# Academich/translation-transformer

Measured on AMD Instinct MI355X. Metric: reactions/sec (SMILES decoded), greedy speculative, higher is better.
Workload: dtype f32

## Files before the change

### include/ttx.h

```cpp
#ifndef TTX_H
#define TTX_H

#include <stdint.h>

#ifdef __cplusplus
extern "C" {
#endif

#define TTX_ABI_VERSION 4

typedef enum ttx_status {
  TTX_OK = 0,
  TTX_ERR_INVALID = -1,
  TTX_ERR_HIP = -2,
  TTX_ERR_NO_DEVICE = -3,
  TTX_ERR_REFERENCE = -4,
  TTX_ERR_NOMEM = -5,
  TTX_ERR_ROW_REPLAY = -6,
  TTX_ERR_MAX_STEPS = -7
} ttx_status;

typedef struct ttx_config {
  int32_t vocab_size;
  int32_t src_vocab_size;
// ... 244 lines not shown
  int32_t max_len, beam_size;
  float   temperature;
  int32_t pad_token, bos_token, eos_token;
  uint64_t seed;
} ttx_sbs_params;
typedef struct ttx_sbs_trace {
  int32_t* d_parent; int32_t* d_token;
  float* d_phi; float* d_g;
} ttx_sbs_trace;
int ttx_sbs_generate(ttx_session* s, const int64_t* d_src, int B, int Ls, const int64_t* d_row_keys, const ttx_sbs_params* p,
                     int64_t* d_out, float* d_logp, float* d_gumbel, const ttx_sbs_trace* trace_or_null,
                     ttx_beam_search_stats* stats, void* stream);

typedef struct ttx_sbs_filter {
  int32_t top_k;
  float   top_p;
} ttx_sbs_filter;
int ttx_sbs_generate_ex(ttx_session* s, const int64_t* d_src, int B, int Ls, const int64_t* d_row_keys, const ttx_sbs_params* p,
                        const ttx_sbs_filter* f_or_null, const int64_t* d_prefix, int ld_prefix, const int32_t* h_prefix_len,
                        int64_t* d_out, float* d_logp, float* d_gumbel, const ttx_sbs_trace* trace_or_null,
                        ttx_beam_search_stats* stats, void* stream);
int ttx_sbs_generate_bias(ttx_session* s, const int64_t* d_src, int B, int Ls, const int64_t* d_row_keys, const ttx_sbs_params* p,
                          const ttx_sbs_filter* f_or_null, const int64_t* d_prefix, int ld_prefix, const int32_t* h_prefix_len,
                          const float* d_bias, int ld_bias, int64_t* d_out, float* d_logp, float* d_gumbel,
                          const ttx_sbs_trace* trace_or_null, ttx_beam_search_stats* stats, void* stream);

typedef struct ttx_sbs_pool_stats {
  int64_t model_calls;
  int64_t running_rows;
  int64_t src_tokens_padded;
  int64_t live_slots;
  double  decode_ms;
  int32_t status;
  int32_t pad_;
  int32_t* d_src_running_rows;
} ttx_sbs_pool_stats;
int ttx_sbs_generate_pool(ttx_session** sessions, int n_sessions, const int64_t* d_src, int S_total, int Ls_all,
                          const int32_t* h_len, const int64_t* d_row_keys, int capacity ,
                          const ttx_sbs_params* p, const ttx_sbs_filter* f_or_null,
                          const int64_t* d_prefix, int ld_prefix, const int32_t* h_prefix_len,
                          int64_t* d_out , float* d_logp, float* d_gumbel ,
                          ttx_sbs_pool_stats* stats, void* stream);

int ttx_greedy_speculative_generate_many(ttx_session** sessions, int n_sessions, int n_batches,
                                         const int64_t* const* d_src, const int* B, const int* Ls,
                                         const ttx_gen_params* p, int64_t* const* d_out, ttx_gen_stats* stats,
                                         void* stream);

int ttx_greedy_speculative_generate_rows(ttx_session** sessions, int n_sessions, int n_batches,
                                         const int64_t* const* d_src, const int* B, const int* Ls,
                                         const ttx_gen_params* p, int64_t* const* d_out, int16_t* const* d_traj,
                                         int32_t* const* d_fin_step, ttx_gen_stats* stats, void* stream);

int ttx_greedy_speculative_generate_pool(ttx_session** sessions, int n_sessions, const int64_t* d_src, int R_total, int Ls_all,
                                         const int32_t* h_len, int capacity, const ttx_gen_params* p, int64_t* d_out,
                                         int16_t* d_traj, int32_t* d_fin_step, ttx_gen_stats* stats, void* stream);

typedef struct ttx_tokenizer ttx_tokenizer;
int  ttx_tokenizer_create(const char* const* tokens, const int32_t* ids, int n, ttx_tokenizer** out);
void ttx_tokenizer_destroy(ttx_tokenizer* t);
int  ttx_tokenizer_encode(const ttx_tokenizer* t, const char* line, int32_t* out, int cap);
int  ttx_tokenizer_encode_batch(const ttx_tokenizer* t, const char* const* lines, int B, int64_t* out, int cap_cols);
int  ttx_tokenizer_decode(const ttx_tokenizer* t, const int64_t* ids, int n, char* out, int cap);

int ttx_debug_step_snapshot(ttx_session* s, int32_t* info, float* h_logits, int32_t* h_act, int32_t* h_front,
                            int32_t* h_gen);

int ttx_last_kernel_profile(ttx_session* s, double* gemm_ms, int64_t* gemm_launches, double* empty_pair_ms);

int ttx_debug_gemm_bench(ttx_session* s, int M, int N, int K, int splits, int variant, int reps, double* us_per_launch,
                         double* max_abs_diff);

int ttx_debug_gemm(ttx_session* s, const float* d_x, int ldx, const float* d_w, int ldw, const float* d_bias, float* d_y, int ldy,
                   const int32_t* d_m, int m_max, int N, int K, int relu, int splits, int64_t slab_stride, int variant, int tiling,
                   int32_t* kernel_id, void* stream);
int ttx_debug_gemm_act(ttx_session* s, const float* d_x, int ldx, const float* d_w, int ldw, const float* d_bias, float* d_y, int ldy,
                       const int32_t* d_m, int m_max, int N, int K, int activation, int splits, int64_t slab_stride, int variant,
                       int tiling, int32_t* kernel_id, void* stream);

int ttx_debug_finish_ln(ttx_session* s, const float* d_slabs, int n_slabs, int64_t slab_stride, const float* d_bias,
                        const float* d_resid, const float* d_g1, const float* d_b1, const float* d_g2, const float* d_b2,
                        const uint8_t* d_row_valid, float* d_y, const int32_t* d_m, int m_max, int d, float eps, void* stream);

int ttx_debug_attn(ttx_session* s, const float* d_q, int ldq, const float* d_k, const float* d_v, int ldkv, float* d_out, int H,
                   float scale, int L, int Lk, const int32_t* d_tok, int pad, const uint8_t* d_key_pad, const int32_t* d_mem_row,
                   const int32_t* d_act_idx, const int32_t* d_front, const int32_t* d_src_of, const int32_t* d_src_len,
                   const float* d_kcache, const float* d_vcache, int64_t cache_seq_stride, const int32_t* d_cache_slot, int gen_ld,
                   int N, int D, int mode, int groups, int n_active, int max_keys, int kernel, int32_t* kernel_id, void* stream);

int ttx_debug_attn_hd(ttx_session* s, const float* d_q, int ldq, const float* d_k, const float* d_v, int ldkv, float* d_out, int H,
                      int head_dim, float scale, int L, int Lk, const int32_t* d_tok, int pad, const uint8_t* d_key_pad,
                      const int32_t* d_mem_row, const int32_t* d_act_idx, const int32_t* d_front, const int32_t* d_src_of,
                      const int32_t* d_src_len, const float* d_kcache, const float* d_vcache, int64_t cache_seq_stride,
                      const int32_t* d_cache_slot, int gen_ld, int N, int D, int mode, int groups, int n_active, int max_keys,
                      int kernel, int32_t* kernel_id, void* stream);

int ttx_debug_attn_as(ttx_session* s, const float* d_q, int ldq, const float* d_k, const float* d_v, int ldkv, float* d_out, int H,
                      int head_dim, float scale, int L, int Lk, const int32_t* d_tok, int pad, const uint8_t* d_key_pad,
                      const int32_t* d_mem_row, const int32_t* d_act_idx, const int32_t* d_front, const int32_t* d_src_of,
                      const int32_t* d_src_len, const float* d_kcache, const float* d_vcache, int64_t cache_seq_stride,
                      const int32_t* d_cache_slot, int gen_ld, int N, int D, int mode, int groups, int n_active, int max_keys,
                      int kernel, int32_t* kernel_id, int sel_N, int sel_D, void* stream);

int ttx_debug_argmax(ttx_session* s, const float* d_logits, int V, int32_t* d_pred, const int32_t* d_m, int m_max, void* stream);

int ttx_debug_sample(ttx_session* s, const float* d_logits, int V, const uint64_t* d_key, const uint32_t* d_sample, int32_t* d_done,
                     const int32_t* d_front, int32_t* d_pred, const int32_t* d_m, int m_max, const ttx_sample_params* p, void* stream);

int ttx_debug_sample_step(ttx_session* s, const float* d_logits, int V, const uint64_t* d_key, const uint32_t* d_sample,
                          const int32_t* d_act_idx, const int32_t* d_front, int B, int N, int D, int n_active, int32_t* d_pred,
                          const int32_t* d_m, const ttx_sample_params* p, void* stream);

int ttx_debug_embed(ttx_session* s, const float* d_table, int V, const float* d_pe, int pe_rows, int d, float* d_x,
                    const int32_t* d_tok, int rows, int L, const int32_t* d_act_idx, const int32_t* d_front, const int32_t* d_gen,
                    int gen_ld, const int32_t* d_drafts, int B, int N, int D, int n_active, int step, void* stream);

typedef struct ttx_debug_accept_args {
  int32_t* d_act_idx; int32_t* d_front; int32_t* d_gen; const int32_t* d_drafts; const int32_t* d_pred; int32_t* d_rec;
  int64_t* d_out; int32_t* d_haspad;
  int16_t* d_traj; int32_t* d_fin_step;
  int32_t* d_rstep; int32_t* d_row_of; int64_t* d_pool_out; int16_t* d_pool_traj; int32_t* d_pool_fin_step;
  int32_t gen_ld, traj_ld, pool_rows, row_rule, pool;
  int32_t B, N, D, Ls, max_len, pad, bos, eos;
  int32_t greedy;
  int32_t threads;
} ttx_debug_accept_args;

int ttx_debug_accept(ttx_session* s, const ttx_debug_accept_args* a, int64_t* state, void* stream);

int ttx_debug_sample_accept(ttx_session* s, const ttx_debug_accept_args* a, int64_t* state, void* stream);

int ttx_debug_sample_step_select(ttx_session* s, const float* d_logits, int V, const uint64_t* d_key, const uint32_t* d_sample,
                                 const int32_t* d_act_idx, const int32_t* d_front, int B, int N, int D, int n_active, int32_t* d_pred,
                                 const int32_t* d_m, const ttx_sample_params* p, const int32_t* d_row_map, int n_rows, void* stream);

typedef struct ttx_debug_prefix {
  const int32_t* d_tok; int32_t ld, n_sources;
  const int32_t* d_len; const int32_t* d_src;
} ttx_debug_prefix;

int ttx_debug_prefix_drafts(ttx_session* s, const int32_t* d_act_idx, const int32_t* d_front, int B, int N, int D, int n_active,
                            int32_t* d_drafts, const int32_t* d_draft0, const ttx_debug_prefix* pfx, int eos_token, int pad_token,
                            int replace_token, void* stream);
int ttx_debug_sample_prefix(ttx_session* s, const float* d_logits, int V, const uint64_t* d_key, const uint32_t* d_sample, int32_t* d_done,
                            const int32_t* d_front, int32_t* d_pred, const int32_t* d_m, int m_max, const ttx_sample_params* p,
                            const ttx_debug_prefix* pfx, void* stream);
int ttx_debug_sample_step_prefix(ttx_session* s, const float* d_logits, int V, const uint64_t* d_key, const uint32_t* d_sample,
                                 const int32_t* d_act_idx, const int32_t* d_front, int B, int N, int D, int n_active, int32_t* d_pred,
                                 const int32_t* d_m, const ttx_sample_params* p, const int32_t* d_row_map, int n_rows,
                                 const ttx_debug_prefix* pfx, void* stream);

int ttx_debug_proposal_drafts(ttx_session* s, const int32_t* d_act_idx, const int32_t* d_front, const int32_t* d_gen, int gen_ld, int B,
                              int N, int D, int n_active, int32_t* d_drafts, const int32_t* d_draft0, const ttx_debug_prefix* proposal,
                              int ctx, int bos_token, int eos_token, int pad_token, int replace_token, void* stream);

int ttx_debug_sample_accept_pool(ttx_session* s, const ttx_debug_accept_args* a, int64_t* state, const int32_t* d_exec_rows, int spread,
                                 void* stream);

typedef struct ttx_debug_pool_fill_args {
  int32_t* d_act_idx; int32_t* d_front; int32_t* d_haspad; int32_t* d_rstep; int32_t* d_row_of; int32_t* d_src_len;
  uint64_t* d_key; uint32_t* d_sample; const int64_t* d_row_keys;
  int32_t* d_gen; int32_t* d_drafts; const int32_t* d_drafts_new; uint8_t* d_src_valid; const uint8_t* d_valid_new;
  float* d_memkv; const float* d_memkv_new; int64_t* d_out;
  int32_t B, N, D, n_active, n_sources, per_src, first_src, Ls_new, Ls_cap, gen_ld, kv_row, max_len, out_rows, bos, pad;
} ttx_debug_pool_fill_args;
int ttx_debug_pool_fill_sample(ttx_session* s, const ttx_debug_pool_fill_args* a, int32_t* result, void* stream);
// ... 177 lines not shown
```

### translation-transformer_amd/_native.py

```python
from __future__ import annotations

import ctypes as C
import os
import subprocess
from pathlib import Path

PKG_DIR = Path(__file__).resolve().parent
CSRC = PKG_DIR / "csrc"
INCLUDE = PKG_DIR.parent / "include"
LIB_PATH = PKG_DIR / "libttx_hip.so"
UNITS = [CSRC / "ttx_api.hip", CSRC / "ttx_gemm.hip", CSRC / "ttx_attn.hip"]
HEADERS = [CSRC / "ttx_internal.h", CSRC / "ttx_common.hip.h", CSRC / "ttx_loop_kernels.hip.h", CSRC / "ttx_metrics.hip.h",
           CSRC / "ttx_score.hip.h", CSRC / "ttx_alternatives.hip.h", CSRC / "ttx_attn_probs.hip.h", CSRC / "ttx_sample.hip.h", CSRC / "ttx_logq.hip.h", CSRC / "ttx_sbs.hip.h", CSRC / "ttx_sbs_pool.hip.h",
           CSRC / "ttx_proposal.hip.h", CSRC / "ttx_logit_bias.hip.h",
           CSRC / "ttx_select.h", CSRC / "ttx_tokenizer.h", CSRC / "ttx_drive.h", CSRC / "ttx_admit.h", INCLUDE / "ttx.h"]
SOURCES = UNITS + HEADERS
OBJ_DIR = CSRC / "build"

TTX_OK, TTX_ERR_INVALID, TTX_ERR_HIP, TTX_ERR_NO_DEVICE, TTX_ERR_REFERENCE, TTX_ERR_NOMEM = 0, -1, -2, -3, -4, -5
TTX_ERR_ROW_REPLAY = -6
TTX_ERR_MAX_STEPS = -7
TTX_ACT_NONE, TTX_ACT_RELU, TTX_ACT_GELU = 0, 1, 2
ACTIVATIONS = {"relu": TTX_ACT_RELU, "gelu": TTX_ACT_GELU}

# ... 221 lines not shown
    "ttx_forward": (C.c_int, [_VP, _VP, _I, _I, _VP, _I, _VP, _VP]),
    "ttx_token_metrics": (C.c_int, [_VP, _VP, _VP, _I, _I, _I, _I, _VP, _VP, _VP, _VP]),
    "ttx_teacher_forced_eval": (C.c_int, [_VP, _VP, _I, _I, _VP, _I, _I, _VP, _VP, _VP, _VP, _VP]),
    "ttx_hypothesis_logprobs": (C.c_int, [_VP, _VP, _VP, _I, _I, _I, _I, _I, _VP, _VP, _VP, _VP, _VP]),
    "ttx_score_hypotheses": (C.c_int, [_VP, _VP, _I, _I, _VP, _I, _I, _I, _I, _VP, _VP, _VP, _VP, _VP, _VP]),
    "ttx_hypothesis_alternatives": (C.c_int, [_VP, _VP, _VP, _I, _I, _I, _I, _I, _I, _VP, _VP, _VP, _VP, _VP, _VP, _VP]),
    "ttx_score_alternatives": (C.c_int, [_VP, _VP, _I, _I, _VP, _I, _I, _I, _I, _I, _VP, _VP, _VP, _VP, _VP, _VP, _VP, _VP]),
    "ttx_hypothesis_logq": (C.c_int, [_VP, _VP, _VP, _I, _I, _I, _I, _I, C.POINTER(Dist), _VP, _VP, _VP, _VP, _VP, _VP, _VP, _VP, _VP]),
    "ttx_score_proposal": (C.c_int, [_VP, _VP, _I, _I, _VP, _I, _I, _I, _I, C.POINTER(Dist), _VP, _VP, _VP, _VP, _VP, _VP, _VP, _VP,
                                    _VP, _VP, _VP, _VP]),
    "ttx_attention_maps": (C.c_int, [_VP, _VP, _I, _I, _VP, _I, _I, _I, _I, _I, _VP, _VP, _VP, _VP, _VP]),
    "ttx_attn_probs_key_limit": (C.c_int, [_I]),
    "ttx_debug_attn_probs": (C.c_int, [_VP, _VP, _I, _VP, _I, _VP, _VP, _VP, _I, _I, _I, _I, _I, _I, C.c_float, _VP, _VP, _VP, _VP]),
    "ttx_make_drafts": (C.c_int, [_VP, _VP, _I, _I, _I, _I, _I, _I, _I, _I, _I, _VP, _VP]),
    "ttx_greedy_speculative_generate": (C.c_int, [_VP, _VP, _I, _I, C.POINTER(GenParams), _VP, C.POINTER(GenStats), _VP]),
    "ttx_greedy_generate": (C.c_int, [_VP, _VP, _I, _I, C.POINTER(GenParams), _VP, C.POINTER(GenStats), _VP]),
    "ttx_sample_generate": (C.c_int, [_VP, _VP, _I, _I, _VP, C.POINTER(SampleParams), _VP, C.POINTER(GenStats), _VP]),
    "ttx_sample_speculative_generate": (C.c_int, [_VP, _VP, _I, _I, _VP, C.POINTER(SampleSpecParams), _VP, C.POINTER(GenStats), _VP]),
    "ttx_sample_generate_prefix": (C.c_int, [_VP, _VP, _I, _I, _VP, C.POINTER(SampleParams), _VP, _I, C.POINTER(C.c_int32), _VP,
                                            C.POINTER(GenStats), _VP]),
    "ttx_sample_speculative_generate_prefix": (C.c_int, [_VP, _VP, _I, _I, _VP, C.POINTER(SampleSpecParams), _VP, _I,
                                                        C.POINTER(C.c_int32), _VP, C.POINTER(GenStats), _VP]),
    "ttx_sample_speculative_generate_pool_prefix": (C.c_int, [C.POINTER(_VP), _I, _VP, _I, _I, C.POINTER(C.c_int32), _VP, _I,
                                                             C.POINTER(SampleSpecParams), _VP, _I, C.POINTER(C.c_int32), _VP,
                                                             C.POINTER(GenStats), _VP]),
    "ttx_sample_speculative_generate_proposal": (C.c_int, [_VP, _VP, _I, _I, _VP, C.POINTER(SampleSpecParams), _VP, _I,
                                                          C.POINTER(C.c_int32), _VP, _I, C.POINTER(C.c_int32), _VP,
                                                          C.POINTER(GenStats), _VP]),
    "ttx_sample_speculative_generate_pool_proposal": (C.c_int, [C.POINTER(_VP), _I, _VP, _I, _I, C.POINTER(C.c_int32), _VP, _I,
                                                               C.POINTER(SampleSpecParams), _VP, _I, C.POINTER(C.c_int32), _VP, _I,
                                                               C.POINTER(C.c_int32), _VP, C.POINTER(GenStats), _VP]),
    "ttx_sample_generate_ex": (C.c_int, [_VP, _VP, _I, _I, _VP, C.POINTER(SampleParams), C.POINTER(SampleOpts), _VP, C.POINTER(GenStats), _VP]),
    "ttx_sample_speculative_generate_ex": (C.c_int, [_VP, _VP, _I, _I, _VP, C.POINTER(SampleSpecParams), C.POINTER(SampleOpts), _VP,
                                                    C.POINTER(GenStats), _VP]),
    "ttx_sample_speculative_generate_pool_ex": (C.c_int, [C.POINTER(_VP), _I, _VP, _I, _I, C.POINTER(C.c_int32), _VP, _I,
                                                         C.POINTER(SampleSpecParams), C.POINTER(SampleOpts), _VP, C.POINTER(GenStats), _VP]),
    "ttx_hypothesis_logq_bias": (C.c_int, [_VP, _VP, _VP, _I, _I, _I, _I, _I, C.POINTER(Dist), _VP, _VP, _I, _I, _VP, _VP, _VP, _VP, _VP,
                                          _VP, _VP, _VP]),
    "ttx_score_proposal_bias": (C.c_int, [_VP, _VP, _I, _I, _VP, _I, _I, _I, _I, C.POINTER(Dist), _VP, _VP, _I, _VP, _VP, _VP, _VP, _VP,
                                         _VP, _VP, _VP, _VP, _VP, _VP]),
    "ttx_sbs_generate_bias": (C.c_int, [_VP, _VP, _I, _I, _VP, C.POINTER(SbsParams), C.POINTER(SbsFilter), _VP, _I, _VP, _VP, _I, _VP, _VP,
                                       _VP, C.POINTER(SbsTrace), C.POINTER(BeamSearchStats), _VP]),
    "ttx_debug_logit_bias_launches": (C.c_int, [_VP]),
    "ttx_debug_logit_bias": (C.c_int, [_VP, _VP, _I, _I, _VP, _VP, _I, _VP, _I, _VP, _VP, _I, _I, _VP]),
    "ttx_greedy_speculative_generate_many": (C.c_int, [C.POINTER(_VP), _I, _I, C.POINTER(_VP), C.POINTER(C.c_int),
                                                      C.POINTER(C.c_int), C.POINTER(GenParams), C.POINTER(_VP),
                                                      C.POINTER(GenStats), _VP]),
    "ttx_greedy_speculative_generate_rows": (C.c_int, [C.POINTER(_VP), _I, _I, C.POINTER(_VP), C.POINTER(C.c_int),
                                                      C.POINTER(C.c_int), C.POINTER(GenParams), C.POINTER(_VP),
                                                      C.POINTER(_VP), C.POINTER(_VP), C.POINTER(GenStats), _VP]),
    "ttx_greedy_speculative_generate_pool": (C.c_int, [C.POINTER(_VP), _I, _VP, _I, _I, C.POINTER(C.c_int32), _I,
                                                      C.POINTER(GenParams), _VP, _VP, _VP, C.POINTER(GenStats), _VP]),
    "ttx_sample_speculative_generate_pool": (C.c_int, [C.POINTER(_VP), _I, _VP, _I, _I, C.POINTER(C.c_int32), _VP, _I,
                                                      C.POINTER(SampleSpecParams), _VP, C.POINTER(GenStats), _VP]),
    "ttx_beam_speculative_generate": (C.c_int, [_VP, _VP, _I, _I, C.POINTER(BeamParams), _VP, C.POINTER(BeamStats), _VP]),
    "ttx_beam_speculative_generate_many": (C.c_int, [C.POINTER(_VP), _I, _I, C.POINTER(_VP), C.POINTER(C.c_int),
                                                    C.POINTER(C.c_int), C.POINTER(BeamParams), C.POINTER(_VP),
                                                    C.POINTER(BeamStats), _VP]),
    "ttx_beam_speculative_generate_pool": (C.c_int, [C.POINTER(_VP), _I, _VP, _I, _I, C.POINTER(C.c_int32), C.POINTER(C.c_int32), _I,
                                                    C.POINTER(C.c_int32), _I, C.POINTER(BeamParams), _VP, _VP, _VP, _I,
                                                    C.POINTER(BeamStats), _VP]),
    "ttx_beam_generate": (C.c_int, [_VP, _VP, _I, _I, C.POINTER(BeamSearchParams), _VP, C.POINTER(BeamSearchStats), _VP]),
    "ttx_sbs_generate": (C.c_int, [_VP, _VP, _I, _I, _VP, C.POINTER(SbsParams), _VP, _VP, _VP, C.POINTER(SbsTrace),
                                  C.POINTER(BeamSearchStats), _VP]),
    "ttx_sbs_generate_ex": (C.c_int, [_VP, _VP, _I, _I, _VP, C.POINTER(SbsParams), C.POINTER(SbsFilter), _VP, _I, _VP, _VP, _VP, _VP,
                                     C.POINTER(SbsTrace), C.POINTER(BeamSearchStats), _VP]),
    "ttx_sbs_generate_pool": (C.c_int, [_VP, _I, _VP, _I, _I, C.POINTER(C.c_int32), _VP, _I, C.POINTER(SbsParams), C.POINTER(SbsFilter),
                                       _VP, _I, _VP, _VP, _VP, _VP, C.POINTER(SbsPoolStats), _VP]),
    "ttx_nucleus_mask": (C.c_int, [_VP, _VP, _I, _I, C.c_float, _I, C.c_float, _VP, _VP]),
    "ttx_accepted_lengths": (C.c_int, [_VP, _VP, _VP, _I, _I, _I, C.c_float, _I, _VP, _VP]),
    "ttx_ragged_topk": (C.c_int, [_VP, _VP, _VP, _I, _I, _I, _VP, _VP, _VP]),
    "ttx_tokenizer_create": (C.c_int, [C.POINTER(C.c_char_p), C.POINTER(C.c_int32), _I, C.POINTER(_VP)]),
    "ttx_tokenizer_destroy": (None, [_VP]),
    "ttx_tokenizer_encode": (C.c_int, [_VP, C.c_char_p, _VP, _I]),
    "ttx_tokenizer_encode_batch": (C.c_int, [_VP, C.POINTER(C.c_char_p), _I, _VP, _I]),
    "ttx_tokenizer_decode": (C.c_int, [_VP, _VP, _I, _VP, _I]),
    "ttx_debug_step_snapshot": (C.c_int, [_VP, C.POINTER(C.c_int32), _VP, _VP, _VP, _VP]),
    "ttx_debug_gemm_bench": (C.c_int, [_VP, _I, _I, _I, _I, _I, _I, C.POINTER(C.c_double), C.POINTER(C.c_double)]),
    "ttx_debug_gemm": (C.c_int, [_VP, _VP, _I, _VP, _I, _VP, _VP, _I, _VP, _I, _I, _I, _I, _I, C.c_int64, _I, _I,
                                 C.POINTER(C.c_int32), _VP]),
    "ttx_debug_gemm_act": (C.c_int, [_VP, _VP, _I, _VP, _I, _VP, _VP, _I, _VP, _I, _I, _I, _I, _I, C.c_int64, _I, _I,
                                     C.POINTER(C.c_int32), _VP]),
    "ttx_debug_finish_ln": (C.c_int, [_VP, _VP, _I, C.c_int64, _VP, _VP, _VP, _VP, _VP, _VP, _VP, _VP, _VP, _I, _I, C.c_float, _VP]),
    "ttx_debug_attn": (C.c_int, [_VP, _VP, _I, _VP, _VP, _I, _VP, _I, C.c_float, _I, _I, _VP, _I, _VP, _VP, _VP, _VP, _VP, _VP, _VP, _VP,
                                 C.c_int64, _VP, _I, _I, _I, _I, _I, _I, _I, _I, C.POINTER(C.c_int32), _VP]),
    "ttx_debug_attn_hd": (C.c_int, [_VP, _VP, _I, _VP, _VP, _I, _VP, _I, _I, C.c_float, _I, _I, _VP, _I, _VP, _VP, _VP, _VP, _VP, _VP, _VP,
                                    _VP, C.c_int64, _VP, _I, _I, _I, _I, _I, _I, _I, _I, C.POINTER(C.c_int32), _VP]),
    "ttx_debug_attn_as": (C.c_int, [_VP, _VP, _I, _VP, _VP, _I, _VP, _I, _I, C.c_float, _I, _I, _VP, _I, _VP, _VP, _VP, _VP, _VP, _VP, _VP,
                                    _VP, C.c_int64, _VP, _I, _I, _I, _I, _I, _I, _I, _I, C.POINTER(C.c_int32), _I, _I, _VP]),
    "ttx_debug_argmax": (C.c_int, [_VP, _VP, _I, _VP, _VP, _I, _VP]),
    "ttx_debug_sample": (C.c_int, [_VP, _VP, _I, _VP, _VP, _VP, _VP, _VP, _VP, _I, C.POINTER(SampleParams), _VP]),
    "ttx_debug_sample_step": (C.c_int, [_VP, _VP, _I, _VP, _VP, _VP, _VP, _I, _I, _I, _I, _VP, _VP, C.POINTER(SampleParams), _VP]),
    "ttx_debug_sample_accept": (C.c_int, [_VP, C.POINTER(DebugAcceptArgs), C.POINTER(C.c_int64), _VP]),
    "ttx_debug_sample_step_select": (C.c_int, [_VP, _VP, _I, _VP, _VP, _VP, _VP, _I, _I, _I, _I, _VP, _VP, C.POINTER(SampleParams),
                                              _VP, _I, _VP]),
    "ttx_debug_prefix_drafts": (C.c_int, [_VP, _VP, _VP, _I, _I, _I, _I, _VP, _VP, C.POINTER(DebugPrefix), _I, _I, _I, _VP]),
    "ttx_debug_proposal_drafts": (C.c_int, [_VP, _VP, _VP, _VP, _I, _I, _I, _I, _I, _VP, _VP, C.POINTER(DebugPrefix), _I, _I, _I, _I,
                                            _I, _VP]),
    "ttx_debug_sample_prefix": (C.c_int, [_VP, _VP, _I, _VP, _VP, _VP, _VP, _VP, _VP, _I, C.POINTER(SampleParams),
                                         C.POINTER(DebugPrefix), _VP]),
    "ttx_debug_sample_step_prefix": (C.c_int, [_VP, _VP, _I, _VP, _VP, _VP, _VP, _I, _I, _I, _I, _VP, _VP, C.POINTER(SampleParams),
                                              _VP, _I, C.POINTER(DebugPrefix), _VP]),
    "ttx_debug_sample_accept_pool": (C.c_int, [_VP, C.POINTER(DebugAcceptArgs), C.POINTER(C.c_int64), _VP, _I, _VP]),
    "ttx_debug_pool_fill_sample": (C.c_int, [_VP, C.POINTER(DebugPoolFillArgs), C.POINTER(C.c_int32), _VP]),
    "ttx_debug_embed": (C.c_int, [_VP, _VP, _I, _VP, _I, _I, _VP, _VP, _I, _I, _VP, _VP, _VP, _I, _VP, _I, _I, _I, _I, _I, _VP]),
    "ttx_debug_accept": (C.c_int, [_VP, C.POINTER(DebugAcceptArgs), C.POINTER(C.c_int64), _VP]),
    "ttx_debug_accept_block": (C.c_int, [_VP, C.POINTER(C.c_int32), _I, _VP]),
    "ttx_debug_bs_prep": (C.c_int, [_VP, C.POINTER(DebugBsPrepArgs), _VP]),
    "ttx_debug_bs_list": (C.c_int, [_VP, C.POINTER(DebugBsListArgs), C.POINTER(C.c_int64), _VP]),
    "ttx_debug_bs_hits": (C.c_int, [_VP, C.POINTER(DebugBsHitsArgs), _VP]),
    "ttx_debug_bs_leaves": (C.c_int, [_VP, C.POINTER(DebugBsLeavesArgs), _VP]),
    "ttx_debug_beam_select": (C.c_int, [_VP, C.POINTER(DebugBeamSelectArgs), _VP]),
    "ttx_debug_beam_step": (C.c_int, [_VP, C.POINTER(DebugBeamStepArgs), _VP]),
    "ttx_debug_sbs_step": (C.c_int, [_VP, C.POINTER(DebugSbsStepArgs), _VP]),
    "ttx_debug_sbs_step_ex": (C.c_int, [_VP, C.POINTER(DebugSbsStepArgs), _I, C.c_float, C.POINTER(DebugPrefix), _I, _VP]),
    "ttx_debug_sbs_step_pool": (C.c_int, [_VP, C.POINTER(DebugSbsStepPoolArgs), _I, _I, C.c_float, C.POINTER(DebugPrefix), _VP]),
    "ttx_debug_sbs_pool": (C.c_int, [_VP, _I, C.POINTER(DebugSbsPoolArgs), C.POINTER(C.c_int64), _VP]),
    "ttx_debug_tree_cache": (C.c_int, [_VP, C.POINTER(DebugTreeCacheArgs), _VP]),
    "ttx_debug_bsp": (C.c_int, [_VP, _I, C.POINTER(DebugBspArgs), C.POINTER(C.c_int64), _VP]),
    "ttx_debug_kvcopy": (C.c_int, [_VP, _VP, _I, _VP, C.c_int64, _VP, _VP, C.c_int64, C.c_int64, _I, _I, _I, _I, _I, _VP]),
    "ttx_debug_kvcopy_split": (C.c_int, [_VP, _VP, _I, _VP, C.c_int64, _VP, _VP, C.c_int64, C.c_int64, _I, _I, _I, _I, _I, _VP, _VP,
                                         C.c_int64, _VP]),
    "ttx_debug_probe_split": (C.c_int, [_VP, _VP, _VP, _VP, _I, _I, _I, _I, _VP, _VP, C.POINTER(C.c_int32), _VP]),
    "ttx_debug_merge_pred": (C.c_int, [_VP, _VP, _VP, _VP, _VP, _I, _I, _I, _I, _VP]),
    "ttx_debug_probe_split_select": (C.c_int, [_VP, _VP, _VP, _VP, _I, _I, _I, _I, _VP, _VP, _VP, _VP, _VP, C.POINTER(C.c_int32), _VP]),
    "ttx_debug_merge_pred_select": (C.c_int, [_VP, _VP, _VP, _VP, _VP, _I, _I, _I, _I, _VP, _VP, _VP]),
    "ttx_debug_kvcopy_select": (C.c_int, [_VP, _VP, _I, _VP, C.c_int64, _VP, _VP, C.c_int64, C.c_int64, _I, _I, _I, _I, _I, _VP, _VP,
                                          C.c_int64, _VP, _VP, _VP]),
    "ttx_debug_embed_select": (C.c_int, [_VP, _VP, _I, _VP, _I, _I, _VP, _VP, _VP, _VP, _I, _VP, _I, _I, _I, _I, _VP, _I, _VP]),
    "ttx_debug_attn_select": (C.c_int, [_VP, _VP, _I, _VP, _VP, _I, _VP, _I, C.c_float, _I, _VP, _I, _VP, _VP, _VP, _VP, _VP, _VP, _VP,
                                        C.c_int64, _VP, _I, _I, _I, _I, _I, _I, _I, _I, C.POINTER(C.c_int32), _VP, _VP, _VP]),
    "ttx_pool_last_counters": (C.c_int, [_VP, C.POINTER(C.c_int64)]),
    "ttx_attn_staged_key_limit": (C.c_int, [_I, _I]),
    "ttx_debug_attn_kernels_seen": (C.c_int, [_VP]),
    "ttx_last_kernel_profile": (C.c_int, [_VP, C.POINTER(C.c_double), C.POINTER(C.c_int64), C.POINTER(C.c_double)]),
}

_lib = None


def hipcc_path() -> str:
    for cand in (os.environ.get("HIPCC"), "/opt/rocm/bin/hipcc", "hipcc"):
        if cand and (os.path.isabs(cand) and os.path.exists(cand) or not os.path.isabs(cand)):
            return cand
    return "hipcc"


def needs_build() -> bool:
    if not LIB_PATH.exists():
        return True
    t = LIB_PATH.stat().st_mtime
    return any(src.stat().st_mtime > t for src in SOURCES)


def build(force: bool = False, verbose: bool = False) -> Path:
    if not force and not needs_build():
        return LIB_PATH
    OBJ_DIR.mkdir(exist_ok=True)
    flags = ["--offload-arch=gfx950", "-O3", "-std=c++17", "-fPIC", f"-I{INCLUDE}"] + os.environ.get("TTX_HIPCC_FLAGS", "").split()
    newest_header = max(h.stat().st_mtime for h in HEADERS)
    jobs, objs = [], []
    for unit in UNITS:
        obj = OBJ_DIR / (unit.stem + ".o")
        objs.append(str(obj))
        if not force and obj.exists() and obj.stat().st_mtime > max(unit.stat().st_mtime, newest_header) \
                and not os.environ.get("TTX_HIPCC_FLAGS"):
# ... 42 lines not shown
```

### translation-transformer_amd/csrc/ttx_api.hip

```cpp
#include "ttx_internal.h"
#include "ttx_admit.h"
#include "ttx_drive.h"
#include "ttx_loop_kernels.hip.h"
#include "ttx_metrics.hip.h"
#include "ttx_score.hip.h"
#include "ttx_alternatives.hip.h"
#include "ttx_attn_probs.hip.h"
#include "ttx_sample.hip.h"
#include "ttx_logit_bias.hip.h"
#include "ttx_logq.hip.h"
#include "ttx_sbs.hip.h"
#include "ttx_sbs_pool.hip.h"
#include "ttx_proposal.hip.h"
#include "ttx_tokenizer.h"

#include <algorithm>
#include <chrono>
#include <cmath>
#include <cstdio>
#include <cstdlib>
#include <cstring>
#include <mutex>
#include <type_traits>

// ... 208 lines not shown
  {
    std::lock_guard<std::mutex> lk(g_retired_mu);
    v.swap(g_retired);
  }
  if (v.empty()) return;
  (void)hipDeviceSynchronize();
  for (void* p : v) (void)hipFree(p);
}

static std::mutex g_stream_mu;
static std::map<int, std::vector<std::pair<int, hipStream_t>>> g_free_streams;
static std::map<hipStream_t, int> g_stream_index;
static int g_streams_made = 0;

static int ensure_own_stream(ttx_session* s) {
  if (s->own_stream) return TTX_OK;
  std::lock_guard<std::mutex> lock(g_stream_mu);
  auto& idle = g_free_streams[s->m->device];
  if (!idle.empty()) {
    auto it = std::min_element(idle.begin(), idle.end());
    s->own_stream = it->second;
    idle.erase(it);
    return TTX_OK;
  }
  HIP_TRY(hipStreamCreateWithFlags(&s->own_stream, hipStreamNonBlocking));
  g_stream_index[s->own_stream] = g_streams_made++;
  return TTX_OK;
}

static void release_own_stream(ttx_session* s) {
  if (!s->own_stream) return;
  std::lock_guard<std::mutex> lock(g_stream_mu);
  g_free_streams[s->m->device].push_back({g_stream_index[s->own_stream], s->own_stream});
  s->own_stream = nullptr;
}

static int ensure(Buf& b, size_t bytes, hipStream_t st) {
  (void)st;
  if (bytes <= b.cap) return TTX_OK;
  if (b.owner_gen) ++*b.owner_gen;
  if (b.p) {
    std::lock_guard<std::mutex> lk(g_retired_mu);
    g_retired.push_back(b.p);
    b.p = nullptr;
    b.cap = 0;
  }
  size_t want = bytes + bytes / 8 + 256;
  if (hipMalloc(&b.p, want) != hipSuccess) return fail(TTX_ERR_NOMEM, "hipMalloc failed for " + std::to_string(want) + " bytes");
  b.cap = want;
  static const bool poison = getenv("TTX_POISON_WORKSPACES") != nullptr && atoi(getenv("TTX_POISON_WORKSPACES")) != 0;
  if (poison) {
    if (hipMemset(b.p, 0xFF, want) != hipSuccess) return fail(TTX_ERR_HIP, "hipMemset (poison) failed");
    (void)hipDeviceSynchronize();
  }
  return TTX_OK;
}

extern "C" int ttx_session_create(ttx_model* m, ttx_session** out) {
  if (!m || !out) return fail(TTX_ERR_INVALID, "null argument");
  HIP_TRY(hipSetDevice(m->device));
  ttx_session* s = new ttx_session();
  s->m = m;
  if (hipHostMalloc((void**)&s->host_info, sizeof(HostInfo), hipHostMallocMapped) != hipSuccess ||
      hipHostMalloc((void**)&s->probe_info, sizeof(ProbeInfo), hipHostMallocMapped) != hipSuccess ||
      hipHostMalloc((void**)&s->host_state, sizeof(DecState), hipHostMallocDefault) != hipSuccess) {
    if (s->host_info) (void)hipHostFree(s->host_info);
    if (s->probe_info) (void)hipHostFree(s->probe_info);
    if (s->host_state) (void)hipHostFree(s->host_state);
    delete s;
    return fail(TTX_ERR_NOMEM, "hipHostMalloc failed");
  }
  std::memset(s->host_info, 0, sizeof(HostInfo));
  std::memset(s->probe_info, 0, sizeof(ProbeInfo));
  HIP_TRY(hipEventCreate(&s->ev_a));
  HIP_TRY(hipEventCreate(&s->ev_b));
  HIP_TRY(hipEventCreate(&s->ev_c));
  HIP_TRY(hipEventCreateWithFlags(&s->ev_done, hipEventDisableTiming));
  s->use_graphs = getenv("TTX_NO_GRAPH") == nullptr;
  const char* pf = getenv("TTX_PROFILE_GEMM");
  s->profile = pf && pf[0] == '1';
  if (const char* e = getenv("TTX_SMALL_ROWS")) s->small_rows = std::max(0, atoi(e));
  if (const char* e = getenv("TTX_FFN2_SLAB_ROWS")) s->ffn2_slab_rows = std::max(0, atoi(e));
  if (const char* e = getenv("TTX_QKV_SMALL_ROWS")) s->qkv_small_rows = std::max(0, atoi(e));
  if (const char* e = getenv("TTX_ATTN_FALLBACK")) s->attn_fallback = atoi(e) != 0;
  if (const char* e = getenv("TTX_ACCEPT_SPREAD")) s->accept_spread = atoi(e) != 0;
  if (const char* e = getenv("TTX_ATTN_ROW")) s->attn_row = atoi(e) != 0 ? 1 : 0;
  s->host_timing = getenv("TTX_HOST_TIMING") != nullptr;
  m->n_sessions++;
  *out = s;
  return TTX_OK;
}

extern "C" void ttx_session_destroy(ttx_session* s) {
  if (!s) return;
  if (s->host_timing && s->host_launches)
    fprintf(stderr, "[ttx host timing] hipGraphLaunch: %lld launches, %.1f us each\n", s->host_launches,
            s->host_launch_us / (double)s->host_launches);
  if (s->host_timing && s->host_captures)
    fprintf(stderr, "[ttx host timing] graphs captured: %lld, %.1f us each\n", s->host_captures,
            s->host_capture_us / (double)s->host_captures);
  if (s->dead) {
    delete s;
    return;
  }
  release_retired();
  (void)hipDeviceSynchronize();
  for (Buf* b : s->all)
    if (b->p) (void)hipFree(b->p);
  if (s->host_info) (void)hipHostFree(s->host_info);
  if (s->probe_info) (void)hipHostFree(s->probe_info);
  if (s->beam_host) (void)hipHostFree(s->beam_host);
  if (s->bp_host) (void)hipHostFree(s->bp_host);
  s->drop_graphs();
  release_own_stream(s);
  if (s->ev_done) (void)hipEventDestroy(s->ev_done);
  if (s->host_state) (void)hipHostFree(s->host_state);
  for (auto& e : s->ev_pool) { (void)hipEventDestroy(e.first); (void)hipEventDestroy(e.second); }
  if (s->ev_a) (void)hipEventDestroy(s->ev_a);
  if (s->ev_b) (void)hipEventDestroy(s->ev_b);
  if (s->ev_c) (void)hipEventDestroy(s->ev_c);
  delete s;
}

static int variant_for_rows(const ttx_session* s, long long rows, bool step) {
  if (!step) return GV_BIG;
  if (rows < s->qkv_small_rows) return GV_SMALL;
  if (rows < s->small_rows) return GV_MID;
  return rows < s->ffn2_slab_rows ? GV_BIG_FFN2_SLABS : GV_BIG;
}
static int variant_qkv(int v) { return v == GV_SMALL ? GV_SMALL : GV_BIG; }
static int variant_dd(int v) { return (v == GV_SMALL || v == GV_MID) ? GV_SMALL : GV_BIG; }
static int variant_ffn1(int v) { return v == GV_SMALL ? GV_SMALL : GV_BIG; }
static int variant_ffn2(int v) { return v == GV_BIG ? GV_BIG : GV_SMALL; }

static int gemm_ln(ttx_session* s, hipStream_t st, const float* X, int ldx, int K, const float* W, const float* bias,
                   const float* resid, const float* g1, const float* b1, const float* g2, const float* b2,
                   const uint8_t* row_valid, float* Y, const int* m_ptr, int Mmax, int variant) {
  const int d = s->m->cfg.embedding_dim;
  const int S = gemm_splits(d, K, m_ptr != nullptr, variant);
  const long long stride = (long long)Mmax * d;
  TTX_TRY(ensure(s->slab, sizeof(float) * (size_t)S * stride, st));
  TTX_TRY(launch_gemm(s, st, X, ldx, W, K, nullptr, s->slab.as<float>(), d, m_ptr, Mmax, d, K, false, S, stride, variant));
  return launch_finish(s, st, s->slab.as<float>(), S, stride, bias, resid, g1, b1, g2, b2, row_valid, Y, m_ptr, Mmax);
}

static int ffn_half(ttx_session* s, hipStream_t st, const LayerW& w, const float* x, size_t n_w, size_t n_b, const float* g2,
                    const float* b2, const uint8_t* row_valid, float* Y, const int* m_ptr, int Mmax, int v_ffn1, int v_ffn2) {
  const ttx_model* m = s->m;
  const int d = m->cfg.embedding_dim, F = m->cfg.feedforward_dim;
  float* hb = s->hbuf.as<float>();
  TTX_TRY(launch_gemm(s, st, x, d, m->p(w.l1_w), d, m->p(w.l1_b), hb, F, m_ptr, Mmax, F, d, m->activation, 0, 0, v_ffn1));
  return gemm_ln(s, st, hb, F, F, m->p(w.l2_w), m->p(w.l2_b), x, m->p(n_w), m->p(n_b), g2, b2, row_valid, Y, m_ptr, Mmax, v_ffn2);
}

static int ensure_acts(ttx_session* s, hipStream_t st, size_t M, int qkv_layers) {
  const ttx_config& c = s->m->cfg;
  const size_t d = c.embedding_dim, F = c.feedforward_dim;
  TTX_TRY(ensure(s->x, M * d * 4, st));
  TTX_TRY(ensure(s->x1, M * d * 4, st));
  TTX_TRY(ensure(s->x2, M * d * 4, st));
  TTX_TRY(ensure(s->xf, M * d * 4, st));
  TTX_TRY(ensure(s->ao, M * d * 4, st));
  TTX_TRY(ensure(s->q2, M * d * 4, st));
  TTX_TRY(ensure(s->hbuf, M * F * 4, st));
  TTX_TRY(ensure(s->qkv, (size_t)qkv_layers * M * 3 * d * 4, st));
  return TTX_OK;
}

static int run_encoder(ttx_session* s, hipStream_t st, const int* tok, const uint8_t* valid, int B, int Ls, float* memory,
                       float* qkv_buf = nullptr) {
  const ttx_model* m = s->m;
  const ttx_config& c = m->cfg;
  const int d = c.embedding_dim, H = c.num_heads;
  const int M = B * Ls;
  const int gv = variant_for_rows(s, M, false);
  TTX_TRY(ensure_acts(s, st, (size_t)M, 1));
  float* x = s->x.as<float>();
  float* x1 = s->x1.as<float>();
  float* qkv = qkv_buf ? qkv_buf : s->qkv.as<float>();
  float* ao = s->ao.as<float>();
  EmbedArgs e{};
  e.table = m->p(m->src_emb); e.pe = m->p(m->pe); e.X = x; e.d = d; e.V = c.src_vocab_size; e.tok = tok; e.rows = M; e.L = Ls;
  hipLaunchKernelGGL((k_embed<false>), dim3(cdiv(M, 4)), dim3(256), 0, st, e);
  HIP_TRY(hipGetLastError());
  for (int l = 0; l < c.num_encoder_layers; ++l) {
    const LayerW& w = m->enc[l];
    const bool last = (l == c.num_encoder_layers - 1);
    TTX_TRY(launch_gemm(s, st, x, d, m->p(w.sa_in_w), d, m->p(w.sa_in_b), qkv, 3 * d, nullptr, M, 3 * d, d, false, 0, 0, gv));
    AttnArgs a{};
    a.q = qkv; a.ldq = 3 * d; a.k = qkv + d; a.v = qkv + 2 * d; a.ldkv = 3 * d; a.out = ao; a.d = d;
    a.scale = 1.0f / sqrtf((float)(d / H)); a.L = Ls; a.tok = tok; a.pad = c.pad_token;
    TTX_TRY(launch_attn(ATT_ENC, s, st, a, B, H, Ls, Ls));
    TTX_TRY(gemm_ln(s, st, ao, d, d, m->p(w.sa_out_w), m->p(w.sa_out_b), x, m->p(w.n1_w), m->p(w.n1_b), nullptr, nullptr,
                    nullptr, x1, nullptr, M, gv));
    TTX_TRY(ffn_half(s, st, w, x1, w.n2_w, w.n2_b, last ? m->p(m->enc_norm_w) : nullptr, last ? m->p(m->enc_norm_b) : nullptr,
                     last ? valid : nullptr, last ? memory : x, nullptr, M, gv, gv));
  }
  return TTX_OK;
}

static int prepare_tokens(hipStream_t st, const int64_t* d_in, int* out, uint8_t* valid, int n, int pad) {
  hipLaunchKernelGGL(k_prepare_tokens, dim3(cdiv(n, 256)), dim3(256), 0, st, d_in, out, valid, n, pad);
  HIP_TRY(hipGetLastError());
  return TTX_OK;
}

static int encode_sources(ttx_session* s, hipStream_t st, const int64_t* d_src, int ld_src, int R, int Ls, uint8_t* valid, float* memkv,
                          float* enc_qkv = nullptr) {
  const ttx_model* m = s->m;
  const int d = m->cfg.embedding_dim, kv_row = m->cfg.num_decoder_layers * 2 * d;
  if (ld_src == 0) {
    TTX_TRY(prepare_tokens(st, d_src, s->tok_src.as<int>(), valid, R * Ls, m->cfg.pad_token));
  } else {
    hipLaunchKernelGGL(k_prepare_tokens_2d, dim3(cdiv(R * Ls, 256)), dim3(256), 0, st, d_src, ld_src, s->tok_src.as<int>(), valid, R, Ls,
                       m->cfg.pad_token);
    HIP_TRY(hipGetLastError());
  }
  TTX_TRY(run_encoder(s, st, s->tok_src.as<int>(), valid, R, Ls, s->memory.as<float>(), enc_qkv));
  return launch_gemm(s, st, s->memory.as<float>(), d, m->p(m->cross_kv_w), d, m->p(m->cross_kv_b), memkv, kv_row, nullptr, R * Ls, kv_row,
                     d, false, 0, 0, variant_for_rows(s, (long long)R * Ls, false));
}

struct Needs {
  hipStream_t st;
  int rc = TTX_OK;
  void operator()(Buf& b, size_t bytes) { if (rc == TTX_OK) rc = ensure(b, bytes, st); }
};

static void need_step_workspaces(ttx_session* s, Needs& need, size_t Mmax, size_t src_rows) {
  const ttx_config& c = s->m->cfg;
  const size_t d = c.embedding_dim, Macts = std::max(Mmax, src_rows);
  need(s->pred, Mmax * 4); need(s->state, sizeof(DecState)); need(s->logits, Mmax * c.vocab_size * 4);
  if (need.rc == TTX_OK) need.rc = ensure_acts(s, need.st, Macts, 1);
  need(s->qkv, std::max((size_t)c.num_decoder_layers * Mmax, src_rows) * 3 * d * 4);
  need(s->slab, sizeof(float) * 16 * Macts * d);
}

extern "C" int ttx_encode_src(ttx_session* s, const int64_t* d_src, int B, int Ls, float* d_memory, void* stream) {
  if (!s || !d_src || !d_memory || B <= 0 || Ls <= 0) return fail(TTX_ERR_INVALID, "bad argument to ttx_encode_src");
  if (Ls > s->m->cfg.max_positions) return fail(TTX_ERR_INVALID, "source longer than the positional table");
  hipStream_t st = (hipStream_t)stream;
  HIP_TRY(hipSetDevice(s->m->device));
  TTX_TRY(ensure(s->tok_src, (size_t)B * Ls * 4, st));
  TTX_TRY(ensure(s->src_valid, (size_t)B * Ls, st));
  TTX_TRY(prepare_tokens(st, d_src, s->tok_src.as<int>(), s->src_valid.as<uint8_t>(), B * Ls, s->m->cfg.pad_token));
  return run_encoder(s, st, s->tok_src.as<int>(), s->src_valid.as<uint8_t>(), B, Ls, d_memory);
}

struct StackRows {
  const int* m_ptr;
  int Mmax;
  int v_qkv, v_dd, v_ffn1, v_ffn2;
  float* qkv;
  long long qkv_layer;
};

template <class SelfAttn, class CrossAttn>
static int run_decoder_stack(ttx_session* s, hipStream_t st, const StackRows& r, SelfAttn&& self_attn, CrossAttn&& cross_attn,
                             float* logits, int stop_layer = -1) {
  const ttx_model* m = s->m;
  const ttx_config& c = m->cfg;
  const int d = c.embedding_dim, V = c.vocab_size, Ld = c.num_decoder_layers;
  float* x = s->x.as<float>();
  float* x1 = s->x1.as<float>();
  float* x2 = s->x2.as<float>();
  float* xf = s->xf.as<float>();
  float* ao = s->ao.as<float>();
  float* q2 = s->q2.as<float>();
  for (int l = 0; l < Ld; ++l) {
    const LayerW& w = m->dec[l];
    const bool last = (l == Ld - 1);
    float* qkv = r.qkv + (size_t)l * r.qkv_layer;
    TTX_TRY(launch_gemm(s, st, x, d, m->p(w.sa_in_w), d, m->p(w.sa_in_b), qkv, 3 * d, r.m_ptr, r.Mmax, 3 * d, d, false, 0, 0, r.v_qkv));
    TTX_TRY(self_attn(l, qkv));
    TTX_TRY(gemm_ln(s, st, ao, d, d, m->p(w.sa_out_w), m->p(w.sa_out_b), x, m->p(w.n1_w), m->p(w.n1_b), nullptr, nullptr,
                    nullptr, x1, r.m_ptr, r.Mmax, r.v_dd));
    TTX_TRY(launch_gemm(s, st, x1, d, m->p(w.ca_in_w), d, m->p(w.ca_in_b), q2, d, r.m_ptr, r.Mmax, d, d, false, 0, 0, r.v_dd));
    TTX_TRY(cross_attn(l));
    if (l == stop_layer) return TTX_OK;
    TTX_TRY(gemm_ln(s, st, ao, d, d, m->p(w.ca_out_w), m->p(w.ca_out_b), x1, m->p(w.n2_w), m->p(w.n2_b), nullptr, nullptr,
                    nullptr, x2, r.m_ptr, r.Mmax, r.v_dd));
    TTX_TRY(ffn_half(s, st, w, x2, w.n3_w, w.n3_b, last ? m->p(m->dec_norm_w) : nullptr, last ? m->p(m->dec_norm_b) : nullptr,
                     nullptr, last ? xf : x, r.m_ptr, r.Mmax, r.v_ffn1, r.v_ffn2));
  }
  return launch_gemm(s, st, xf, d, m->p(m->cls_w), d, m->p(m->cls_b), logits, V, r.m_ptr, r.Mmax, V, d, false, 0, 0, r.v_dd);
}

struct AttnTap {
  int layer;
  const int* length;
  float* heads;
  float* mean;
  int* align;
};

static int launch_attn_probs(ttx_session* s, hipStream_t st, const AttnProbsArgs& a, int head_dim);

static int run_decoder_full(ttx_session* s, hipStream_t st, const int* tok, int R, int Lt, const float* memory,
                            const uint8_t* mem_pad, const int* mem_row, int Rm, int Ls, float* logits,
                            const AttnTap* tap = nullptr) {
  const ttx_model* m = s->m;
  const ttx_config& c = m->cfg;
  const int d = c.embedding_dim, H = c.num_heads;
  const int M = R * Lt, Mk = Rm * Ls;
  const int gv = variant_for_rows(s, M, false);
  TTX_TRY(ensure_acts(s, st, (size_t)M, 1));
  TTX_TRY(ensure(s->ckv, (size_t)Mk * 2 * d * 4, st));
  float* ao = s->ao.as<float>();
  float* ckv = s->ckv.as<float>();
  const float scale = 1.0f / sqrtf((float)(d / H));
  EmbedArgs e{};
  e.table = m->p(m->tgt_emb); e.pe = m->p(m->pe); e.X = s->x.as<float>(); e.d = d; e.V = c.vocab_size; e.tok = tok; e.rows = M; e.L = Lt;
  hipLaunchKernelGGL((k_embed<false>), dim3(cdiv(M, 4)), dim3(256), 0, st, e);
  HIP_TRY(hipGetLastError());
  const StackRows rows{nullptr, M, gv, gv, gv, gv, s->qkv.as<float>(), 0};
  return run_decoder_stack(s, st, rows,
      [&](int, float* qkv) -> int {
        AttnArgs a{};
        a.q = qkv; a.ldq = 3 * d; a.k = qkv + d; a.v = qkv + 2 * d; a.ldkv = 3 * d; a.out = ao; a.d = d; a.scale = scale;
        a.L = Lt; a.tok = tok; a.pad = c.pad_token;
        return launch_attn(ATT_FULL_SELF, s, st, a, R, H, Lt, Lt);
      },
      [&](int l) -> int {
        const LayerW& w = m->dec[l];
        TTX_TRY(launch_gemm(s, st, memory, d, m->p(w.ca_in_w) + (size_t)d * d, d, m->p(w.ca_in_b) + d, ckv, 2 * d, nullptr, Mk,
                            2 * d, d, false, 0, 0, gv));
        if (tap && l == tap->layer) {
          AttnProbsArgs pa{};
          pa.q = s->q2.as<float>(); pa.ldq = d; pa.k = ckv; pa.ldkv = 2 * d; pa.key_pad = mem_pad; pa.mem_row = mem_row;
          pa.length = tap->length; pa.heads = tap->heads; pa.mean = tap->mean; pa.align = tap->align;
          pa.R = R; pa.Rm = Rm; pa.H = H; pa.T = Lt; pa.Ls = Ls; pa.scale = scale;
          return launch_attn_probs(s, st, pa, d / H);
        }
        AttnArgs ca{};
        ca.q = s->q2.as<float>(); ca.ldq = d; ca.k = ckv; ca.v = ckv + d; ca.ldkv = 2 * d; ca.out = ao; ca.d = d; ca.scale = scale;
        ca.L = Lt; ca.Lk = Ls; ca.key_pad = mem_pad; ca.mem_row = mem_row;
        return launch_attn(ATT_FULL_CROSS, s, st, ca, R, H, Lt, Ls);
      },
      logits, tap ? tap->layer : -1);
}

extern "C" int ttx_decode_tgt(ttx_session* s, const int64_t* d_tgt, int R, int Lt, const float* d_memory,
                              const uint8_t* d_mem_pad, const int32_t* d_mem_row, int Rm, int Ls, float* d_logits,
                              void* stream) {
  if (!s || !d_tgt || !d_memory || !d_mem_pad || !d_logits || R <= 0 || Lt <= 0 || Rm <= 0 || Ls <= 0)
    return fail(TTX_ERR_INVALID, "bad argument to ttx_decode_tgt");
  if (!d_mem_row && Rm != R) return fail(TTX_ERR_INVALID, "without a row map the memory must have one row per decoder row");
  if (Lt > s->m->cfg.max_positions) return fail(TTX_ERR_INVALID, "target longer than the positional table");
  hipStream_t st = (hipStream_t)stream;
  HIP_TRY(hipSetDevice(s->m->device));
  TTX_TRY(ensure(s->tok_tgt, (size_t)R * Lt * 4, st));
  TTX_TRY(prepare_tokens(st, d_tgt, s->tok_tgt.as<int>(), nullptr, R * Lt, s->m->cfg.pad_token));
  return run_decoder_full(s, st, s->tok_tgt.as<int>(), R, Lt, d_memory, d_mem_pad, d_mem_row, Rm, Ls, d_logits);
}

__global__ void k_invert_mask(const uint8_t* valid, uint8_t* pad, int n) {
  const int i = blockIdx.x * blockDim.x + threadIdx.x;
  if (i < n) pad[i] = valid[i] ? 0 : 1;
}

extern "C" int ttx_forward(ttx_session* s, const int64_t* d_src, int B, int Ls, const int64_t* d_tgt, int Lt,
                           float* d_logits, void* stream) {
  if (!s || !d_src || !d_tgt || !d_logits || B <= 0 || Ls <= 0 || Lt <= 0) return fail(TTX_ERR_INVALID, "bad argument to ttx_forward");
  hipStream_t st = (hipStream_t)stream;
  HIP_TRY(hipSetDevice(s->m->device));
  const int d = s->m->cfg.embedding_dim;
  TTX_TRY(ensure(s->memory, (size_t)B * Ls * d * 4, st));
  TTX_TRY(ensure(s->mem_pad_tmp, (size_t)B * Ls, st));
  TTX_TRY(ttx_encode_src(s, d_src, B, Ls, s->memory.as<float>(), stream));
  hipLaunchKernelGGL(k_invert_mask, dim3(cdiv(B * Ls, 256)), dim3(256), 0, st, s->src_valid.as<uint8_t>(),
                     s->mem_pad_tmp.as<uint8_t>(), B * Ls);
  HIP_TRY(hipGetLastError());
  return ttx_decode_tgt(s, d_tgt, B, Lt, s->memory.as<float>(), s->mem_pad_tmp.as<uint8_t>(), nullptr, B, Ls, d_logits, stream);
}

static int session_required(const char* fn) {
  int n = 0;
  if (hipGetDeviceCount(&n) != hipSuccess || n <= 0)
    return fail(TTX_ERR_NO_DEVICE, "no HIP device visible; libttx_hip has no CPU fallback");
  return fail(TTX_ERR_INVALID, std::string("bad argument to ") + fn + ": null session");
}

static int check_metric_shapes(const ttx_session* s, int B, int Lt, int V, const char* fn) {
  if (B <= 0 || Lt < 2 || V <= 0) return fail(TTX_ERR_INVALID, std::string("bad argument to ") + fn + ": B > 0, Lt >= 2, V > 0");
  if (V > MET_MAX_V) return fail(TTX_ERR_INVALID, std::string(fn) + ": vocabulary larger than 1024");
  if ((long long)B * (Lt - 1) >= (1LL << 24))
    return fail(TTX_ERR_INVALID, std::string(fn) + ": more than 2^24 positions in one call");
  if (Lt - 1 > s->m->cfg.max_positions) return fail(TTX_ERR_INVALID, std::string(fn) + ": target longer than the positional table");
  return TTX_OK;
}

static int launch_metrics(ttx_session* s, hipStream_t st, const float* logits, const int64_t* tgt, int B, int Lt, int V, int eos,
                          int64_t* pred, float* nll, float* out3) {
  const int M = B * (Lt - 1);
  if (!pred) {
    TTX_TRY(ensure(s->ev_pred, (size_t)M * sizeof(int64_t), st));
    pred = s->ev_pred.as<int64_t>();
  }
// ... 370 lines not shown
}

static int launch_sample(hipStream_t st, const SampleArgs& a) {
  const dim3 grid(cdiv(a.M, 4)), block(256);
  if (a.V <= 64) hipLaunchKernelGGL((k_sample<1>), grid, block, 0, st, a);
  else if (a.V <= 128) hipLaunchKernelGGL((k_sample<2>), grid, block, 0, st, a);
  else if (a.V <= 256) hipLaunchKernelGGL((k_sample<4>), grid, block, 0, st, a);
  else if (a.V <= 512) hipLaunchKernelGGL((k_sample<8>), grid, block, 0, st, a);
  else hipLaunchKernelGGL((k_sample<16>), grid, block, 0, st, a);
  HIP_TRY(hipGetLastError());
  return TTX_OK;
}

static int launch_sample_step(hipStream_t st, const SampleStepArgs& a) {
  const dim3 grid(cdiv(a.M, 4)), block(256);
  if (a.V <= 64) hipLaunchKernelGGL((k_sample_step<1>), grid, block, 0, st, a);
  else if (a.V <= 128) hipLaunchKernelGGL((k_sample_step<2>), grid, block, 0, st, a);
  else if (a.V <= 256) hipLaunchKernelGGL((k_sample_step<4>), grid, block, 0, st, a);
  else if (a.V <= 512) hipLaunchKernelGGL((k_sample_step<8>), grid, block, 0, st, a);
  else hipLaunchKernelGGL((k_sample_step<16>), grid, block, 0, st, a);
  HIP_TRY(hipGetLastError());
  return TTX_OK;
}

static int launch_prefix_drafts_args(hipStream_t st, const PrefixDraftsArgs& a, int B) {
  hipLaunchKernelGGL(k_prefix_drafts, dim3(cdiv(B, 4)), dim3(256), 0, st, a);
  HIP_TRY(hipGetLastError());
  return TTX_OK;
}

static int launch_proposal_drafts_args(hipStream_t st, const ProposalDraftsArgs& a, int B) {
  hipLaunchKernelGGL(k_proposal_drafts, dim3(cdiv(B, 4)), dim3(256), 0, st, a);
  HIP_TRY(hipGetLastError());
  return TTX_OK;
}

static const PrefixTab& step_tab(const StepCtx& k) { return k.sample.pfx.tok ? k.sample.pfx : k.prop; }

static int launch_prefix_drafts(ttx_session* s, hipStream_t st, const StepCtx& k) {
  if (k.prop.tok && k.want_sample_step) {
    ProposalDraftsArgs a{};
    a.st = s->state.as<DecState>(); a.act_idx = s->act_idx.as<int>(); a.front = s->front.as<int>();
    a.gen = s->gen.as<int>(); a.gen_ld = k.gen_ld;
    a.drafts = s->drafts.as<int>(); a.N = k.N; a.D = k.D; a.draft0 = k.pfx_draft0; a.tab = k.prop;
    a.bos = k.p.bos_token; a.eos = k.p.eos_token; a.pad = k.p.pad_token; a.repl = k.p.replace_token; a.ctx = k.prop_ctx;
    return launch_proposal_drafts_args(st, a, k.B);
  }
  if (!k.sample.pfx.tok || !k.want_sample_step) return TTX_OK;
  PrefixDraftsArgs a{};
  a.st = s->state.as<DecState>(); a.act_idx = s->act_idx.as<int>(); a.front = s->front.as<int>();
  a.drafts = s->drafts.as<int>(); a.N = k.N; a.D = k.D; a.draft0 = k.pfx_draft0; a.pfx = k.sample.pfx;
  a.eos = k.p.eos_token; a.pad = k.p.pad_token; a.repl = k.p.replace_token;
  return launch_prefix_drafts_args(st, a, k.B);
}

static int run_step(ttx_session* s, hipStream_t st, const StepCtx& k, int kcap) {
  const ttx_model* m = s->m;
  const ttx_config& c = m->cfg;
  const int d = c.embedding_dim, H = c.num_heads, V = c.vocab_size, Ld = c.num_decoder_layers;
  const int D1 = k.D + 1;
  const int RPS = step_rps(k.N, k.D);
  const int Mmax = k.B * RPS;
  DecState* dst = k.st_ov ? k.st_ov : s->state.as<DecState>();
  const int* act = k.act_ov ? k.act_ov : s->act_idx.as<int>();
  const int* m_ptr = &dst->m_rows;
  float* ao = s->ao.as<float>();
  float* logits = s->logits.as<float>();
  const float scale = 1.0f / sqrtf((float)(d / H));
  const long long cache_seq = (long long)k.Lc * d;
  const long long cache_layer = (long long)k.B * cache_seq;

  struct AttnSel {
    ttx_session* s;
    AttnSel(ttx_session* s_, int N, int D) : s(s_) { s->attn_sel_N = N; s->attn_sel_D = D; }
    ~AttnSel() { s->attn_sel_N = 0; s->attn_sel_D = 0; }
  } attn_sel(s, k.sel_N, k.sel_D);
  EmbedArgs e{};
  e.table = m->p(m->tgt_emb); e.pe = m->p(m->pe); e.X = s->x.as<float>(); e.d = d; e.V = c.vocab_size;
  e.st = dst; e.act_idx = act; e.front = s->front.as<int>(); e.gen = s->gen.as<int>(); e.gen_ld = k.gen_ld;
  e.drafts = s->drafts.as<int>(); e.N = k.N; e.D = k.D; e.row_map = k.row_map;
  hipLaunchKernelGGL((k_embed<true>), dim3(cdiv(Mmax, 4)), dim3(256), 0, st, e);
  HIP_TRY(hipGetLastError());

  const StackRows rows{m_ptr, Mmax, variant_qkv(k.variant), variant_dd(k.variant), variant_ffn1(k.variant), variant_ffn2(k.variant),
                       k.qkv_ov ? k.qkv_ov : s->qkv.as<float>(), (long long)Mmax * 3 * d};
  TTX_TRY(run_decoder_stack(s, st, rows,
      [&](int l, float* qkv) -> int {
        AttnArgs a{};
        a.q = qkv; a.ldq = 3 * d; a.k = qkv + d; a.v = qkv + 2 * d; a.ldkv = 3 * d; a.out = ao; a.d = d; a.scale = scale;
        a.tok = s->gen.as<int>(); a.pad = c.pad_token; a.st = dst; a.act_idx = act; a.front = s->front.as<int>();
        a.kcache = (k.kcache ? k.kcache : s->kcache.as<float>()) + (size_t)l * cache_layer;
        a.vcache = (k.vcache ? k.vcache : s->vcache.as<float>()) + (size_t)l * cache_layer;
        a.cache_seq_stride = cache_seq; a.gen_ld = k.gen_ld; a.N = k.N; a.D = k.D; a.cache_slot = k.cache_slot;
        a.row_base = k.row_base; a.draft_mask = k.draft_mask;
        return launch_attn(ATT_STEP_SELF, s, st, a, k.B, H, RPS, kcap, k.N, D1);
      },
      [&](int l) -> int {
        AttnArgs ca{};
        ca.q = s->q2.as<float>(); ca.ldq = d; ca.k = s->memkv.as<float>() + (size_t)l * 2 * d; ca.v = ca.k + d; ca.ldkv = Ld * 2 * d;
        ca.out = ao; ca.d = d; ca.scale = scale; ca.Lk = k.Ls; ca.key_pad = s->src_valid.as<uint8_t>();
        ca.st = dst; ca.act_idx = act; ca.front = s->front.as<int>(); ca.N = k.N; ca.D = k.D;
        ca.src_of = k.src_of; ca.src_len = k.src_len; ca.row_base = k.row_base; ca.draft_mask = k.draft_mask;
        return launch_attn(ATT_STEP_CROSS, s, st, ca, k.B, H, RPS, k.Ls, k.N, D1);
      },
      logits));
  if (k.bias.val) {
    LogitBiasArgs b{};
    b.logits = logits; b.V = V; b.m_ptr = m_ptr; b.M = Mmax; b.tab = k.bias; b.rows_per_src = 1;
    if (!k.want_sample) { b.act_idx = act; b.row_map = k.row_map; b.N = k.N; b.D = k.D; }
    TTX_TRY(launch_logit_bias(st, b, !k.want_sample));
    s->logit_bias_launches += 1;
  }
  if (k.want_sample) {
    SampleArgs a = k.sample;
    a.logits = logits; a.V = V; a.pred = s->pred.as<int>(); a.m_ptr = m_ptr; a.M = Mmax;
    return launch_sample(st, a);
  }
  if (k.want_sample_step) {
    SampleStepArgs a{};
    a.logits = logits; a.V = V; a.pred = k.pred_ov ? k.pred_ov : s->pred.as<int>(); a.m_ptr = m_ptr; a.M = Mmax;
    a.key = k.sample.key; a.sample = k.sample.sample; a.prm = k.sample.prm;
    a.act_idx = act; a.front = s->front.as<int>(); a.N = k.N; a.D = k.D; a.row_map = k.row_map; a.pfx = k.sample.pfx;
    return launch_sample_step(st, a);
  }
  if (k.want_argmax) {
    hipLaunchKernelGGL(k_argmax, dim3(cdiv(Mmax, 4)), dim3(256), 0, st, logits, V, k.pred_ov ? k.pred_ov : s->pred.as<int>(), m_ptr, Mmax);
    HIP_TRY(hipGetLastError());
  }
  return TTX_OK;
}

struct GenCtx {
  StepCtx k;
  LoopArgs la;
  KvCopyArgs kc;
};

static int launch_accept(hipStream_t st, const LoopArgs& la, int threads) {
  if (la.blk) {
    hipLaunchKernelGGL(k_accept_slots, dim3(cdiv(la.B, ACCEPT_SLOT_WAVES)), dim3(ACCEPT_SLOT_WAVES * 64), 0, st, la);
    HIP_TRY(hipGetLastError());
    hipLaunchKernelGGL(k_accept_finish, dim3(1), dim3(ACCEPT_THREADS), 0, st, la);
  } else {
    hipLaunchKernelGGL(k_accept, dim3(1), dim3(threads ? threads : (la.B > 256 ? ACCEPT_THREADS : 256)), 0, st, la);
  }
  HIP_TRY(hipGetLastError());
  return TTX_OK;
}

static int launch_sample_accept(hipStream_t st, const LoopArgs& la) {
  if (la.blk) {
    hipLaunchKernelGGL(k_sample_accept_slots, dim3(cdiv(la.B, ACCEPT_SLOT_WAVES)), dim3(ACCEPT_SLOT_WAVES * 64), 0, st, la);
    HIP_TRY(hipGetLastError());
    hipLaunchKernelGGL(k_accept_finish, dim3(1), dim3(ACCEPT_THREADS), 0, st, la);
  } else {
    hipLaunchKernelGGL(k_sample_accept, dim3(1), dim3(la.B > 256 ? ACCEPT_THREADS : 256), 0, st, la);
  }
  HIP_TRY(hipGetLastError());
  return TTX_OK;
}

static int accept_blk_when(ttx_session* s, hipStream_t st, int B, bool spread, AcceptBlk** out) {
  *out = nullptr;
  if (!spread || B <= 256) return TTX_OK;
  const void* before = s->accept_blk.p;
  TTX_TRY(ensure(s->accept_blk, sizeof(AcceptBlk), st));
  if (s->accept_blk.p != before) HIP_TRY(hipMemsetAsync(s->accept_blk.p, 0, sizeof(AcceptBlk), st));
  *out = s->accept_blk.as<AcceptBlk>();
// ... 2577 lines not shown
  if (!tokens || !ids || n <= 0 || !out) return fail(TTX_ERR_INVALID, "bad argument to ttx_tokenizer_create");
  ttx_tokenizer* t = new ttx_tokenizer();
  int32_t max_id = -1;
  for (int i = 0; i < n; ++i) max_id = std::max(max_id, ids[i]);
  t->dec.assign((size_t)max_id + 1, std::string());
  for (int i = 0; i < n; ++i) {
    if (!tokens[i] || ids[i] < 0) { delete t; return fail(TTX_ERR_INVALID, "vocabulary entry with a null token or negative id"); }
    t->enc[tokens[i]] = ids[i];
    t->dec[ids[i]] = tokens[i];
  }
  *out = t;
  return TTX_OK;
}

extern "C" void ttx_tokenizer_destroy(ttx_tokenizer* t) { delete t; }

extern "C" int ttx_tokenizer_encode(const ttx_tokenizer* t, const char* line, int32_t* out, int cap) {
  if (!t || !line) return fail(TTX_ERR_INVALID, "null argument to ttx_tokenizer_encode");
  int n = 0;
  auto put = [&](int32_t id) { if (out && n < cap) out[n] = id; ++n; };
  put(t->bos);
  std::string piece;
  ttxtok::split(line, std::strlen(line), [&](const char* p, size_t len) {
    piece.assign(p, len);
    auto it = t->enc.find(piece);
    put(it == t->enc.end() ? t->unk : it->second);
  });
  put(t->eos);
  return n;
}

extern "C" int ttx_tokenizer_encode_batch(const ttx_tokenizer* t, const char* const* lines, int B, int64_t* out, int cap_cols) {
  if (!t || !lines || B <= 0 || !out || cap_cols <= 0) return fail(TTX_ERR_INVALID, "bad argument to ttx_tokenizer_encode_batch");
  std::vector<int32_t> row((size_t)cap_cols);
  int width = 0;
  for (int b = 0; b < B; ++b) {
    const int n = ttx_tokenizer_encode(t, lines[b], row.data(), cap_cols);
    if (n < 0) return n;
    width = std::max(width, n);
    if (n <= cap_cols) {
      for (int i = 0; i < n; ++i) out[(size_t)b * cap_cols + i] = row[i];
      for (int i = n; i < cap_cols; ++i) out[(size_t)b * cap_cols + i] = t->pad;
    }
  }
  return width <= cap_cols ? width : -width;
}

extern "C" int ttx_tokenizer_decode(const ttx_tokenizer* t, const int64_t* ids, int n, char* out, int cap) {
  if (!t || (!ids && n > 0)) return fail(TTX_ERR_INVALID, "null argument to ttx_tokenizer_decode");
  size_t len = 0;
  for (int i = 0; i < n; ++i) {
    const int64_t id = ids[i];
    if (id != t->bos && id != t->eos && id != t->pad) {
      if (id < 0 || (size_t)id >= t->dec.size() || (t->dec[id].empty() && t->enc.find("") == t->enc.end()))
        return fail(TTX_ERR_REFERENCE, "token id outside the vocabulary (KeyError in the reference)");
      const std::string& tok = t->dec[id];
      for (char ch : tok) { if (out && (int)len + 1 < cap) out[len] = ch; ++len; }
    }
    if (id == t->eos) break;
  }
  if (out && cap > 0) out[std::min(len, (size_t)cap - 1)] = '\0';
  return (int)len;
}

extern "C" int ttx_debug_gemm_bench(ttx_session* s, int M, int N, int K, int splits, int variant, int reps, double* us_per_launch,
                                    double* max_abs_diff) {
  return gemm_bench(s, M, N, K, splits, variant, reps, us_per_launch, max_abs_diff);
}

extern "C" int ttx_debug_gemm_act(ttx_session* s, const float* d_x, int ldx, const float* d_w, int ldw, const float* d_bias, float* d_y,
                                  int ldy, const int32_t* d_m, int m_max, int N, int K, int activation, int splits, int64_t slab_stride,
                                  int variant, int tiling, int32_t* kernel_id, void* stream) {
  return gemm_debug(s, d_x, ldx, d_w, ldw, d_bias, d_y, ldy, d_m, m_max, N, K, activation, splits, (long long)slab_stride, variant,
                    tiling, kernel_id, reinterpret_cast<hipStream_t>(stream));
}

extern "C" int ttx_debug_gemm(ttx_session* s, const float* d_x, int ldx, const float* d_w, int ldw, const float* d_bias, float* d_y,
                              int ldy, const int32_t* d_m, int m_max, int N, int K, int relu, int splits, int64_t slab_stride,
                              int variant, int tiling, int32_t* kernel_id, void* stream) {
  return ttx_debug_gemm_act(s, d_x, ldx, d_w, ldw, d_bias, d_y, ldy, d_m, m_max, N, K, relu ? TTX_ACT_RELU : TTX_ACT_NONE, splits,
                            slab_stride, variant, tiling, kernel_id, stream);
}

extern "C" int ttx_debug_finish_ln(ttx_session* s, const float* d_slabs, int n_slabs, int64_t slab_stride, const float* d_bias,
                                   const float* d_resid, const float* d_g1, const float* d_b1, const float* d_g2, const float* d_b2,
                                   const uint8_t* d_row_valid, float* d_y, const int32_t* d_m, int m_max, int d, float eps,
                                   void* stream) {
  return finish_debug(s, d_slabs, n_slabs, (long long)slab_stride, d_bias, d_resid, d_g1, d_b1, d_g2, d_b2, d_row_valid, d_y, d_m,
                      m_max, d, eps, reinterpret_cast<hipStream_t>(stream));
}

extern "C" int ttx_debug_attn_hd(ttx_session* s, const float* d_q, int ldq, const float* d_k, const float* d_v, int ldkv, float* d_out,
                                 int H, int head_dim, float scale, int L, int Lk, const int32_t* d_tok, int pad, const uint8_t* d_key_pad,
                                 const int32_t* d_mem_row, const int32_t* d_act_idx, const int32_t* d_front, const int32_t* d_src_of,
                                 const int32_t* d_src_len, const float* d_kcache, const float* d_vcache, int64_t cache_seq_stride,
                                 const int32_t* d_cache_slot, int gen_ld, int N, int D, int mode, int groups, int n_active, int max_keys,
                                 int kernel, int32_t* kernel_id, void* stream) {
  AttnArgs a{};
  a.q = d_q; a.ldq = ldq; a.k = d_k; a.v = d_v; a.ldkv = ldkv; a.out = d_out; a.scale = scale; a.L = L; a.Lk = Lk;
  a.tok = d_tok; a.pad = pad; a.key_pad = d_key_pad; a.mem_row = d_mem_row; a.act_idx = d_act_idx; a.front = d_front;
  a.src_of = d_src_of; a.src_len = d_src_len; a.kcache = d_kcache; a.vcache = d_vcache; a.cache_seq_stride = (long long)cache_seq_stride;
  a.cache_slot = d_cache_slot; a.gen_ld = gen_ld; a.N = N; a.D = D;
  return attn_debug(s, a, H, head_dim, mode, groups, n_active, max_keys, kernel, kernel_id, reinterpret_cast<hipStream_t>(stream));
}

extern "C" int ttx_debug_attn_as(ttx_session* s, const float* d_q, int ldq, const float* d_k, const float* d_v, int ldkv, float* d_out,
                                 int H, int head_dim, float scale, int L, int Lk, const int32_t* d_tok, int pad, const uint8_t* d_key_pad,
                                 const int32_t* d_mem_row, const int32_t* d_act_idx, const int32_t* d_front, const int32_t* d_src_of,
                                 const int32_t* d_src_len, const float* d_kcache, const float* d_vcache, int64_t cache_seq_stride,
                                 const int32_t* d_cache_slot, int gen_ld, int N, int D, int mode, int groups, int n_active, int max_keys,
                                 int kernel, int32_t* kernel_id, int sel_N, int sel_D, void* stream) {
  if (!s) return fail(TTX_ERR_INVALID, "null session");
  if (sel_N < 1 || sel_D < 0) return fail(TTX_ERR_INVALID, "ttx_debug_attn_as: the layout to choose as needs N >= 1 and D >= 0");
  s->attn_sel_N = sel_N; s->attn_sel_D = sel_D;
  const int rc = ttx_debug_attn_hd(s, d_q, ldq, d_k, d_v, ldkv, d_out, H, head_dim, scale, L, Lk, d_tok, pad, d_key_pad, d_mem_row, d_act_idx,
                                   d_front, d_src_of, d_src_len, d_kcache, d_vcache, cache_seq_stride, d_cache_slot, gen_ld, N, D, mode,
                                   groups, n_active, max_keys, kernel, kernel_id, stream);
  s->attn_sel_N = 0; s->attn_sel_D = 0;
  return rc;
}

extern "C" int ttx_debug_attn(ttx_session* s, const float* d_q, int ldq, const float* d_k, const float* d_v, int ldkv, float* d_out,
                              int H, float scale, int L, int Lk, const int32_t* d_tok, int pad, const uint8_t* d_key_pad,
                              const int32_t* d_mem_row, const int32_t* d_act_idx, const int32_t* d_front, const int32_t* d_src_of,
                              const int32_t* d_src_len, const float* d_kcache, const float* d_vcache, int64_t cache_seq_stride,
                              const int32_t* d_cache_slot, int gen_ld, int N, int D, int mode, int groups, int n_active, int max_keys,
                              int kernel, int32_t* kernel_id, void* stream) {
  return ttx_debug_attn_hd(s, d_q, ldq, d_k, d_v, ldkv, d_out, H, 32, scale, L, Lk, d_tok, pad, d_key_pad, d_mem_row, d_act_idx, d_front,
                           d_src_of, d_src_len, d_kcache, d_vcache, cache_seq_stride, d_cache_slot, gen_ld, N, D, mode, groups, n_active,
                           max_keys, kernel, kernel_id, stream);
}

static int dbg_check_select(const std::string& who, const int32_t* d_row_base, const int32_t* d_draft_mask, int n, int N, int D,
                            hipStream_t st, std::vector<int32_t>* mask_out, int* total) {
  *total = 0;
  if (!d_row_base || !d_draft_mask) return fail(TTX_ERR_INVALID, who + ": row_base and draft_mask are required");
  if (N < 1 || N > 32 || D < 1) return fail(TTX_ERR_INVALID, who + ": draft select needs 1 <= N <= 32 and D >= 1");
  std::vector<int32_t> base((size_t)std::max(n, 1)), mask((size_t)std::max(n, 1));
  if (n > 0) {
    HIP_TRY(hipStreamSynchronize(st));
    HIP_TRY(hipMemcpy(base.data(), d_row_base, (size_t)n * 4, hipMemcpyDeviceToHost));
    HIP_TRY(hipMemcpy(mask.data(), d_draft_mask, (size_t)n * 4, hipMemcpyDeviceToHost));
  }
  int sum = 0;
  for (int p = 0; p < n; ++p) {
    const unsigned m = (unsigned)mask[p];
    if (m == 0u || (N < 32 && (m >> N))) return fail(TTX_ERR_INVALID, who + ": a listed slot's draft mask must be a non-zero subset of the N drafts");
    if (base[p] != sum) return fail(TTX_ERR_INVALID, who + ": row_base must be the exclusive prefix sum of 1 + D * popcount(mask)");
    sum += step_sel_rows(m, D);
  }
  mask.resize((size_t)n);
  if (mask_out) *mask_out = mask;
  *total = sum;
  return TTX_OK;
}

extern "C" int ttx_debug_attn_select(ttx_session* s, const float* d_q, int ldq, const float* d_k, const float* d_v, int ldkv, float* d_out,
                                     int H, float scale, int Lk, const int32_t* d_tok, int pad, const uint8_t* d_key_pad,
                                     const int32_t* d_act_idx, const int32_t* d_front, const int32_t* d_src_of, const int32_t* d_src_len,
                                     const float* d_kcache, const float* d_vcache, int64_t cache_seq_stride, const int32_t* d_cache_slot,
                                     int gen_ld, int N, int D, int mode, int groups, int n_active, int max_keys, int kernel,
                                     int32_t* kernel_id, const int32_t* d_row_base, const int32_t* d_draft_mask, void* stream) {
  if (!s) return fail(TTX_ERR_INVALID, "null session");
  if (mode != ATT_STEP_SELF && mode != ATT_STEP_CROSS) return fail(TTX_ERR_INVALID, "ttx_debug_attn_select: a step mode (3 or 4) is required");
  if (kernel != 0 && kernel != AK_ATTN3 && kernel != AK_ATTN3S)
    return fail(TTX_ERR_INVALID, "ttx_debug_attn_select: draft select runs on k_attn3 (3) or k_attn3s (4); 0 chooses between them");
// ... 1263 lines not shown
```

### translation-transformer_amd/csrc/ttx_gemm.hip

```cpp
#include "ttx_internal.h"

#include <algorithm>
#include <cmath>

namespace ttx {

template <int WGM, int WGN, bool GELU = false>
__global__ __launch_bounds__(64 * WGM * WGN) void k_gemm_tn(GemmArgs a) {
  constexpr int NT = 64 * WGM * WGN;
  constexpr int BM = 32 * WGM, BN = 32 * WGN, BK = 32, LDT = BK + 4;
  constexpr int RPP = NT / 8;
  constexpr int AP = BM / RPP, BP = BN / RPP;
  static_assert(AP >= 1 && BP >= 1, "tile too small for the thread count");
  __shared__ __attribute__((aligned(16))) float As[BM * LDT];
  __shared__ __attribute__((aligned(16))) float Bs[BN * LDT];

  const int M = a.m_ptr ? *a.m_ptr : a.M;
  const int m0 = blockIdx.y * BM, n0 = blockIdx.x * BN;
  if (m0 >= M) return;
  const int kbeg = blockIdx.z * a.k_per_split;
  const int kend = min(a.K, kbeg + a.k_per_split);

  const int t = threadIdx.x;
  const int lr = t >> 3, lc = (t & 7) * 4;
// ... 407 lines not shown
      __syncthreads();
      i += 2;
    }
  };
  int s = 0;
  if constexpr (ALT) {
    for (; s + 1 < n_slices; s += 2) {
      slice(a00, a10, b00, b10, s == 0 ? 0 : 2);
      slice(b00, b10, a00, a10, s == 0 ? 1 : 2);
    }
  }
  f32x16 c00, c10;
  if constexpr (!ALT) {
    for (; s < n_slices; ++s) {
      slice(a00, a10, b00, b10, 0);
      fold_values(t00, a00, s == 0 ? 1 : 2, 0, 16); fold_values(t10, a10, s == 0 ? 1 : 2, 0, 16);
    }
    c00 = t00; c10 = t10;
  } else if (n_slices == 1) {
    slice(a00, a10, b00, b10, 0);
    c00 = a00; c10 = a10;
  } else {
    if (s < n_slices) {
      slice(a00, a10, b00, b10, 2);
      fold_values(t00, a00, 2, 0, 16); fold_values(t10, a10, 2, 0, 16);
    } else {
      fold_values(t00, b00, 2, 0, 16); fold_values(t10, b10, 2, 0, 16);
    }
    c00 = t00; c10 = t10;
  }

  if constexpr (GELU) bias0 = (!a.raw && a.bias) ? a.bias[min(bcol, a.N - 1)] : 0.f;
  float* Y = a.Y + (a.raw ? (size_t)bz * a.slab_stride : 0);
  const float lo = a.relu ? 0.f : -INFINITY;
  auto store_tile = [&](const f32x16& c, int tm) {
    const int col = n0 + wn * WN + r;
    float val[16];
#pragma unroll
    for (int v = 0; v < 16; ++v) val[v] = gemm_act<GELU>(c[v] + bias0, lo);
    const int row0 = m0 + wm * 64 + tm * 32 + 4 * h;
    float* yp = Y + (size_t)row0 * a.ldy + col;
    if (m0 + BM <= M && n0 + BN <= a.N) {
#pragma unroll
      for (int v = 0; v < 16; ++v) yp[(size_t)((v & 3) + 8 * (v >> 2)) * a.ldy] = val[v];
    } else if (col < a.N) {
      const int rows_left = M - row0;
#pragma unroll
      for (int v = 0; v < 16; ++v) {
        const int dr = (v & 3) + 8 * (v >> 2);
        if (dr < rows_left) yp[(size_t)dr * a.ldy] = val[v];
      }
    }
  };
  store_tile(c00, 0);
  store_tile(c10, 1);
}

__device__ __forceinline__ bool tile_of_workgroup(int n_tiles, int nbx, int nby, int& bx, int& by, int& slab) {
  const int lin = blockIdx.x + gridDim.x * (blockIdx.y + gridDim.y * blockIdx.z);
  if (lin >= n_tiles) return false;
  const int xb = n_tiles >> 3, xr = n_tiles & 7, xcd = lin & 7;
  const int v = xcd * xb + min(xcd, xr) + (lin >> 3);
  slab = v / (nbx * nby);
  const int rem = v - slab * (nbx * nby);
  bx = rem % nbx; by = rem / nbx;
  return true;
}

template <int NT, bool GELU = false>
__global__ __launch_bounds__(256) __attribute__((amdgpu_waves_per_eu(2, 2))) void k_gemm24(GemmArgs a) {
  __shared__ __attribute__((aligned(16))) float smem[G24_SMEM_FLOATS];
  const int M = a.m_ptr ? *a.m_ptr : a.M;
  const int nby = (M + 127) >> 7, nbx = (a.N + 63) >> 6;
  const int mid_tiles = nby * nbx * (int)gridDim.z;
  if (a.big_min_tiles > 0 && mid_tiles >= a.big_min_tiles) {
    int bx, by, slab;
    if (!tile_of_workgroup(mid_tiles, nbx, nby, bx, by, slab)) return;
    g4_body<NT == 4, GELU>(a, M, bx, by, slab, smem);
  } else {
    g2_body<NT, GELU>(a, M, blockIdx.x, blockIdx.y, blockIdx.z, smem);
  }
}

template <bool GELU = false>
__global__ __launch_bounds__(256) __attribute__((amdgpu_waves_per_eu(1, 4))) void k_gemm3(GemmArgs a) {
  constexpr int KW = 64;
  __shared__ __attribute__((aligned(16))) float part[4][32 * 33];
  const int M = a.m_ptr ? *a.m_ptr : a.M;
  const int m0 = blockIdx.y * 32, n0 = blockIdx.x * 32;
  if (m0 >= M) return;
  const int t = threadIdx.x, wave = t >> 6, lane = t & 63;
  const int r = lane & 31, h = lane >> 5;
  const int kbeg = blockIdx.z * a.k_per_split + wave * KW;
  const float* xp = a.X + (size_t)min(m0 + r, M - 1) * a.ldx + kbeg + 4 * h;
  const float* wp = a.W + (size_t)min(n0 + r, a.N - 1) * a.ldw + kbeg + 4 * h;
  f32x16 acc;
#pragma unroll
  for (int i = 0; i < 16; ++i) acc[i] = 0.f;
  typedef float f32x4 __attribute__((ext_vector_type(4)));
  f32x4 av[KW / 8], bv[KW / 8];
#pragma unroll
  for (int g = 0; g < KW / 8; ++g) {
    av[g] = *reinterpret_cast<const f32x4*>(xp + 8 * g);
    bv[g] = *reinterpret_cast<const f32x4*>(wp + 8 * g);
  }
  asm volatile("" : "+v"(av[0]), "+v"(av[1]), "+v"(av[2]), "+v"(av[3]), "+v"(av[4]), "+v"(av[5]), "+v"(av[6]), "+v"(av[7]),
                    "+v"(bv[0]), "+v"(bv[1]), "+v"(bv[2]), "+v"(bv[3]), "+v"(bv[4]), "+v"(bv[5]), "+v"(bv[6]), "+v"(bv[7]));
#pragma unroll
  for (int g = 0; g < KW / 8; ++g) {
    acc = __builtin_amdgcn_mfma_f32_32x32x2f32(av[g].x, bv[g].x, acc, 0, 0, 0);
    acc = __builtin_amdgcn_mfma_f32_32x32x2f32(av[g].y, bv[g].y, acc, 0, 0, 0);
    acc = __builtin_amdgcn_mfma_f32_32x32x2f32(av[g].z, bv[g].z, acc, 0, 0, 0);
    acc = __builtin_amdgcn_mfma_f32_32x32x2f32(av[g].w, bv[g].w, acc, 0, 0, 0);
  }
#pragma unroll
  for (int v = 0; v < 16; ++v) part[wave][((v & 3) + 8 * (v >> 2) + 4 * h) * 33 + r] = acc[v];
  __syncthreads();
  const int row = t >> 3, c0 = (t & 7) * 4;
  float4 o;
  float* op = &o.x;
#pragma unroll
  for (int i = 0; i < 4; ++i) {
    const int e = row * 33 + c0 + i;
    op[i] = ((part[0][e] + part[1][e]) + part[2][e]) + part[3][e];
  }
  const int grow = m0 + row, gcol = n0 + c0;
  if (grow < M && gcol < a.N) {
    float* Y = a.Y + (a.raw ? (size_t)blockIdx.z * a.slab_stride : 0) + (size_t)grow * a.ldy + gcol;
    const float lo = a.relu ? 0.f : -INFINITY;
    if (gcol + 3 < a.N && (a.ldy & 3) == 0) {
      float4 bb = make_float4(0.f, 0.f, 0.f, 0.f);
      if (!a.raw && a.bias) bb = *reinterpret_cast<const float4*>(a.bias + gcol);
      o.x = gemm_act<GELU>(o.x + bb.x, lo); o.y = gemm_act<GELU>(o.y + bb.y, lo); o.z = gemm_act<GELU>(o.z + bb.z, lo); o.w = gemm_act<GELU>(o.w + bb.w, lo);
      *reinterpret_cast<float4*>(Y) = o;
    } else {
      for (int i = 0; i < 4 && gcol + i < a.N; ++i) {
        const float bb = (!a.raw && a.bias) ? a.bias[gcol + i] : 0.f;
        Y[i] = gemm_act<GELU>(op[i] + bb, lo);
      }
    }
  }
}

template <int VPL>
__device__ __forceinline__ void ln_inplace(float (&x)[VPL], const float* g, const float* b, int c0, int d, float eps) {
  float s = 0.f;
#pragma unroll
  for (int i = 0; i < VPL; ++i) s += x[i];
  const float mean = wave_sum(s) / (float)d;
  float q = 0.f;
#pragma unroll
  for (int i = 0; i < VPL; ++i) { const float t = x[i] - mean; q += t * t; }
  const float var = wave_sum(q) / (float)d;
  const float rstd = 1.0f / sqrtf(var + eps);
#pragma unroll
  for (int i = 0; i < VPL; ++i) x[i] = (x[i] - mean) * rstd * g[c0 + i] + b[c0 + i];
}

template <int VPL>
__global__ __launch_bounds__(256) void k_finish_ln(FinishArgs a) {
  const int M = a.m_ptr ? *a.m_ptr : a.M;
  const int row = blockIdx.x * 4 + (threadIdx.x >> 6);
  if (row >= M) return;
  const int lane = threadIdx.x & 63;
  const int c0 = lane * VPL;
  float x[VPL];
  const size_t off = (size_t)row * a.d + c0;
  if constexpr (VPL == 4) {
    if (a.n_slabs == 1 || a.n_slabs == 8) {
      const float4 r4 = *reinterpret_cast<const float4*>(a.resid + off);
      const float4 b4 = *reinterpret_cast<const float4*>(a.bias + c0);
      float4 tsum = *reinterpret_cast<const float4*>(a.slabs + off);
      if (a.n_slabs == 8) {
        float4 p[7];
#pragma unroll
        for (int s = 0; s < 7; ++s) p[s] = *reinterpret_cast<const float4*>(a.slabs + (size_t)(s + 1) * a.slab_stride + off);
#pragma unroll
        for (int s = 0; s < 7; ++s) { tsum.x += p[s].x; tsum.y += p[s].y; tsum.z += p[s].z; tsum.w += p[s].w; }
      }
      const float4 g1 = *reinterpret_cast<const float4*>(a.g1 + c0);
      const float4 e1 = *reinterpret_cast<const float4*>(a.b1 + c0);
      const float* g2p = a.g2 ? a.g2 : a.g1;
      const float* e2p = a.g2 ? a.b2 : a.b1;
      const float4 g2 = *reinterpret_cast<const float4*>(g2p + c0);
      const float4 e2 = *reinterpret_cast<const float4*>(e2p + c0);
      const uint8_t valid = a.row_valid ? a.row_valid[row] : (uint8_t)1;
      x[0] = (r4.x + b4.x) + tsum.x; x[1] = (r4.y + b4.y) + tsum.y; x[2] = (r4.z + b4.z) + tsum.z; x[3] = (r4.w + b4.w) + tsum.w;
      const float ga[4] = {g1.x, g1.y, g1.z, g1.w}, ea[4] = {e1.x, e1.y, e1.z, e1.w};
      ln_inplace<4>(x, ga, ea, 0, a.d, a.eps);
      if (a.g2) {
        const float gb[4] = {g2.x, g2.y, g2.z, g2.w}, eb[4] = {e2.x, e2.y, e2.z, e2.w};
        ln_inplace<4>(x, gb, eb, 0, a.d, a.eps);
      }
      const bool keep = valid != 0;
      *reinterpret_cast<float4*>(a.Y + off) = make_float4(keep ? x[0] : 0.f, keep ? x[1] : 0.f, keep ? x[2] : 0.f, keep ? x[3] : 0.f);
      return;
    }
  }
  float tsum[VPL];
#pragma unroll
  for (int i = 0; i < VPL; ++i) tsum[i] = a.slabs[off + i];
  for (int s = 1; s < a.n_slabs; ++s) {
    const float* p = a.slabs + (size_t)s * a.slab_stride + off;
#pragma unroll
    for (int i = 0; i < VPL; ++i) tsum[i] += p[i];
  }
#pragma unroll
  for (int i = 0; i < VPL; ++i) x[i] = (a.resid[off + i] + a.bias[c0 + i]) + tsum[i];
  ln_inplace<VPL>(x, a.g1, a.b1, c0, a.d, a.eps);
  if (a.g2) ln_inplace<VPL>(x, a.g2, a.b2, c0, a.d, a.eps);
  const bool keep = a.row_valid ? (a.row_valid[row] != 0) : true;
#pragma unroll
  for (int i = 0; i < VPL; ++i) a.Y[off + i] = keep ? x[i] : 0.f;
}


int gemm_slice_k(int K) {
  if (K == 64 || K == 128) return 64;
  if (K % 256) return 0;
  return K >= 2048 ? 256 : 64;
}

static bool use_gemm3(bool step, int variant, int N, int K) {
  return step && variant == GV_SMALL && K == 256 && N <= 768;
}

int gemm_splits(int N, int K, bool step, int variant) {
  (void)N;
  if (step && variant == GV_SMALL && gemm_slice_k(K) == 256 && K / 256 <= 16) return K / 256;
  return 1;
}

int launch_gemm(ttx_session* s, hipStream_t st, const float* X, int ldx, const float* W, int ldw, const float* bias,
                float* Y, int ldy, const int* m_ptr, int Mmax, int N, int K, int act, int splits, long long slab_stride,
                int variant) {
  if (act != TTX_ACT_NONE && act != TTX_ACT_RELU && act != TTX_ACT_GELU) return fail(TTX_ERR_INVALID, "GEMM activation must be a ttx_activation");
  if (Mmax <= 0) return TTX_OK;
  if (K % 32) return fail(TTX_ERR_INVALID, "GEMM K must be a multiple of 32");
  GemmArgs a;
  a.X = X; a.ldx = ldx; a.W = W; a.ldw = ldw; a.bias = bias; a.Y = Y; a.ldy = ldy; a.m_ptr = m_ptr;
  a.M = Mmax; a.N = N; a.K = K; a.relu = act == TTX_ACT_RELU ? 1 : 0;
  a.raw = splits > 0 ? 1 : 0;
  const int S = splits > 0 ? splits : 1;
  a.k_per_split = K / S;
  a.slab_stride = slab_stride;
  a.slice_k = gemm_slice_k(K);
  if (K % S) return fail(TTX_ERR_INVALID, "GEMM K must be a multiple of the slab count");
  if (a.raw && act != TTX_ACT_NONE) return fail(TTX_ERR_INVALID, "raw split-K slabs take no activation");
  if (a.slice_k && a.k_per_split % a.slice_k) return fail(TTX_ERR_INVALID, "split-K slabs must be whole canonical slices");
  if (a.slice_k && a.k_per_split != 64 && a.k_per_split != 128 && a.k_per_split % 256)
    return fail(TTX_ERR_INVALID, "split-K slabs must be 64, 128 or a multiple of 256 deep");
  if (!a.slice_k && a.k_per_split % 32) return fail(TTX_ERR_INVALID, "split-K slabs must be a multiple of 32 deep");
  a.big_min_tiles = 0;
  hipEvent_t e1 = nullptr;
  if (s->profile) {
    if (s->ev_used == s->ev_pool.size()) {
      hipEvent_t a0, a1;
      HIP_TRY(hipEventCreate(&a0));
      HIP_TRY(hipEventCreate(&a1));
      s->ev_pool.push_back({a0, a1});
    }
    HIP_TRY(hipEventRecord(s->ev_pool[s->ev_used].first, st));
    e1 = s->ev_pool[s->ev_used].second;
    s->ev_used++;
  }
  const bool step = (m_ptr != nullptr);
  const bool gelu = act == TTX_ACT_GELU;
  s->last_gemm_big_min_tiles = 0;
  if (use_gemm3(step, variant, N, K) && S == 1) {
    s->last_gemm_kernel = GK_GEMM3;
    if (gelu) hipLaunchKernelGGL((k_gemm3<true>), dim3(cdiv(N, 32), cdiv(Mmax, 32), 1), dim3(256), 0, st, a);
    else hipLaunchKernelGGL((k_gemm3<false>), dim3(cdiv(N, 32), cdiv(Mmax, 32), 1), dim3(256), 0, st, a);
  } else if (a.slice_k == 0) {
    s->last_gemm_kernel = GK_GEMM_TN;
    if (gelu) hipLaunchKernelGGL((k_gemm_tn<2, 2, true>), dim3(cdiv(N, 64), cdiv(Mmax, 64), S), dim3(256), 0, st, a);
    else hipLaunchKernelGGL((k_gemm_tn<2, 2>), dim3(cdiv(N, 64), cdiv(Mmax, 64), S), dim3(256), 0, st, a);
  } else if (a.k_per_split % 256 == 0 && !(step && variant == GV_SMALL)) {
    a.big_min_tiles = K >= 2048 ? std::max(1, s->big_min_tiles / 3) : (N >= 2048 ? 2 * s->big_min_tiles : s->big_min_tiles);
    if (s->big_min_tiles == 0) a.big_min_tiles = 0;
    dim3 grid(cdiv(N, 64), cdiv(Mmax, 64), S);
    s->last_gemm_kernel = a.k_per_split == 256 ? GK_GEMM24_4 : GK_GEMM24_0;
    s->last_gemm_big_min_tiles = a.big_min_tiles;
    if (gelu) {
      if (a.k_per_split == 256) hipLaunchKernelGGL((k_gemm24<4, true>), grid, dim3(256), 0, st, a);
      else hipLaunchKernelGGL((k_gemm24<0, true>), grid, dim3(256), 0, st, a);
    } else if (a.k_per_split == 256) hipLaunchKernelGGL((k_gemm24<4>), grid, dim3(256), 0, st, a);
    else hipLaunchKernelGGL((k_gemm24<0>), grid, dim3(256), 0, st, a);
  } else {
    dim3 grid(cdiv(N, 64), cdiv(Mmax, 64), S);
    s->last_gemm_kernel = a.k_per_split == 64 ? GK_GEMM2_1 : a.k_per_split == 128 ? GK_GEMM2_2 : a.k_per_split == 256 ? GK_GEMM2_4 : GK_GEMM2_0;
    if (gelu) switch (a.k_per_split) {
      case 64: hipLaunchKernelGGL((k_gemm2<1, true>), grid, dim3(256), 0, st, a); break;
      case 128: hipLaunchKernelGGL((k_gemm2<2, true>), grid, dim3(256), 0, st, a); break;
      case 256: hipLaunchKernelGGL((k_gemm2<4, true>), grid, dim3(256), 0, st, a); break;
      default: hipLaunchKernelGGL((k_gemm2<0, true>), grid, dim3(256), 0, st, a); break;
    }
    else switch (a.k_per_split) {
      case 64: hipLaunchKernelGGL((k_gemm2<1>), grid, dim3(256), 0, st, a); break;
      case 128: hipLaunchKernelGGL((k_gemm2<2>), grid, dim3(256), 0, st, a); break;
      case 256: hipLaunchKernelGGL((k_gemm2<4>), grid, dim3(256), 0, st, a); break;
      default: hipLaunchKernelGGL((k_gemm2<0>), grid, dim3(256), 0, st, a); break;
    }
  }
  if (e1) HIP_TRY(hipEventRecord(e1, st));
  HIP_TRY(hipGetLastError());
  return TTX_OK;
}

int launch_finish(ttx_session* s, hipStream_t st, const float* slabs, int n_slabs, long long slab_stride, const float* bias,
                  const float* resid, const float* g1, const float* b1, const float* g2, const float* b2,
                  const uint8_t* row_valid, float* Y, const int* m_ptr, int Mmax) {
  const ttx_config& c = s->m->cfg;
  return launch_finish_d(st, slabs, n_slabs, slab_stride, bias, resid, g1, b1, g2, b2, row_valid, Y, m_ptr, Mmax, c.embedding_dim,
                         c.layer_norm_eps);
}

int launch_finish_d(hipStream_t st, const float* slabs, int n_slabs, long long slab_stride, const float* bias, const float* resid,
                    const float* g1, const float* b1, const float* g2, const float* b2, const uint8_t* row_valid, float* Y,
                    const int* m_ptr, int Mmax, int d, float eps) {
  if (Mmax <= 0) return TTX_OK;
  FinishArgs a;
  a.slabs = slabs; a.n_slabs = n_slabs; a.slab_stride = slab_stride; a.bias = bias; a.resid = resid;
  a.g1 = g1; a.b1 = b1; a.g2 = g2; a.b2 = b2; a.row_valid = row_valid; a.Y = Y; a.m_ptr = m_ptr; a.M = Mmax;
  a.d = d; a.eps = eps;
  dim3 grid(cdiv(Mmax, 4));
  switch (d / 64) {
    case 1: hipLaunchKernelGGL((k_finish_ln<1>), grid, dim3(256), 0, st, a); break;
    case 2: hipLaunchKernelGGL((k_finish_ln<2>), grid, dim3(256), 0, st, a); break;
    case 4: hipLaunchKernelGGL((k_finish_ln<4>), grid, dim3(256), 0, st, a); break;
    case 8: hipLaunchKernelGGL((k_finish_ln<8>), grid, dim3(256), 0, st, a); break;
    default: hipLaunchKernelGGL((k_finish_ln<16>), grid, dim3(256), 0, st, a); break;
  }
  HIP_TRY(hipGetLastError());
  return TTX_OK;
}

int gemm_bench(ttx_session* s, int M, int N, int K, int splits, int variant, int reps, double* us_per_launch, double* max_abs_diff) {
  if (!s || M <= 0 || N <= 0 || K <= 0 || gemm_slice_k(K) == 0 || reps <= 0) return fail(TTX_ERR_INVALID, "bad argument to ttx_debug_gemm_bench");
  HIP_TRY(hipSetDevice(s->m->device));
  const int S = splits > 0 ? splits : 1;
  const int slice = gemm_slice_k(K);
  if (K % S || (K / S) % std::max(slice, 64)) return fail(TTX_ERR_INVALID, "K / splits must be a whole number of canonical slices");
  if (variant == 3 && (K != 256 || S != 1)) return fail(TTX_ERR_INVALID, "variant 3 serves K = 256 without slabs");
  std::vector<float> hx((size_t)M * K), hw((size_t)N * K), hb(N);
  uint64_t z = 0x9E3779B97F4A7C15ull;
  auto rnd = [&]() { z ^= z << 13; z ^= z >> 7; z ^= z << 17; return (float)((z >> 40) & 0xffff) / 65536.f - 0.5f; };
  for (auto& v : hx) v = rnd();
  for (auto& v : hw) v = rnd() * 0.125f;
  for (auto& v : hb) v = rnd();
  float *dx = nullptr, *dw = nullptr, *db = nullptr, *dy = nullptr, *dref = nullptr;
  int* dm = nullptr;
  HIP_TRY(hipMalloc(&dx, hx.size() * 4));
// ... 51 lines not shown
  }
  s->big_min_tiles = keep_min; s->profile = was_profile;
  if (e0) (void)hipEventDestroy(e0);
  if (e1) (void)hipEventDestroy(e1);
  (void)hipStreamDestroy(st);
  (void)hipFree(dx); (void)hipFree(dw); (void)hipFree(db); (void)hipFree(dy); (void)hipFree(dref); (void)hipFree(dm);
  return rc;
}

static bool aligned16(const void* p) { return (reinterpret_cast<uintptr_t>(p) & 15) == 0; }

static int debug_live_rows(const int32_t* d_m, int m_max, hipStream_t st, int* M) {
  *M = m_max;
  if (!d_m) return TTX_OK;
  int32_t m = -1;
  HIP_TRY(hipStreamSynchronize(st));
  HIP_TRY(hipMemcpy(&m, d_m, 4, hipMemcpyDeviceToHost));
  if (m < 0 || m > m_max) return fail(TTX_ERR_INVALID, "live row count on the device is outside [0, m_max]");
  *M = m;
  return TTX_OK;
}

int gemm_debug(ttx_session* s, const float* d_x, int ldx, const float* d_w, int ldw, const float* d_bias, float* d_y, int ldy,
               const int32_t* d_m, int m_max, int N, int K, int act, int splits, long long slab_stride, int variant, int tiling,
               int32_t* kernel_id, hipStream_t st) {
  if (!s || !d_x || !d_w || !d_y) return fail(TTX_ERR_INVALID, "null argument to ttx_debug_gemm");
  if (act != TTX_ACT_NONE && act != TTX_ACT_RELU && act != TTX_ACT_GELU) return fail(TTX_ERR_INVALID, "ttx_debug_gemm_act: activation is 0 (none), 1 (ReLU) or 2 (GELU)");
  if (m_max <= 0 || N <= 0 || K <= 0 || splits < 0) return fail(TTX_ERR_INVALID, "ttx_debug_gemm: m_max, N, K must be positive and splits >= 0");
  if (K % 32) return fail(TTX_ERR_INVALID, "ttx_debug_gemm: K must be a multiple of 32");
  if (variant < GV_BIG || variant > GV_MID || tiling < 0 || tiling > 2) return fail(TTX_ERR_INVALID, "ttx_debug_gemm: variant is 0..3, tiling 0..2");
  if (ldx < K || ldw < K || ldy < N) return fail(TTX_ERR_INVALID, "ttx_debug_gemm: leading dimensions must cover K (X, W) and N (Y)");
  if ((ldx & 3) || (ldw & 3) || !aligned16(d_x) || !aligned16(d_w))
    return fail(TTX_ERR_INVALID, "ttx_debug_gemm: X and W are read as float4 (16-byte aligned pointers, ldx and ldw multiples of 4)");
  if ((d_bias && !aligned16(d_bias)) || ((ldy & 3) == 0 && !aligned16(d_y)))
    return fail(TTX_ERR_INVALID, "ttx_debug_gemm: bias, and Y when ldy is a multiple of 4, must be 16-byte aligned");
  const int S = splits > 0 ? splits : 1;
  const int slice = gemm_slice_k(K);
  if (K % S) return fail(TTX_ERR_INVALID, "ttx_debug_gemm: K must be a multiple of splits");
  const int kps = K / S;
  if (slice ? (kps % slice != 0 || (kps != 64 && kps != 128 && kps % 256 != 0)) : (kps % 32 != 0))
    return fail(TTX_ERR_INVALID, "ttx_debug_gemm: slabs must be whole canonical slices (64, 128 or a multiple of 256 k's; 32 without slices)");
  if (S > 1 && (slab_stride < (long long)(m_max - 1) * ldy + N || ((slab_stride & 3) && (ldy & 3) == 0)))
    return fail(TTX_ERR_INVALID, "ttx_debug_gemm: slab_stride must cover one [m_max, ldy] slab");
  HIP_TRY(hipSetDevice(s->m->device));
  int M = 0;
  TTX_TRY(debug_live_rows(d_m, m_max, st, &M));
  const bool was_profile = s->profile;
  const int keep_min = s->big_min_tiles;
  s->profile = false;
  if (tiling == 1) s->big_min_tiles = 0;
  else if (tiling == 2) s->big_min_tiles = 1;
  const int rc = launch_gemm(s, st, d_x, ldx, d_w, ldw, d_bias, d_y, ldy, d_m, m_max, N, K, act, splits, slab_stride, variant);
  s->big_min_tiles = keep_min; s->profile = was_profile;
  if (rc != TTX_OK) return rc;
  if (kernel_id) {
    int id = s->last_gemm_kernel;
    if (id == GK_GEMM24_4 || id == GK_GEMM24_0) {
      const int mid_tiles = ((M + 127) >> 7) * ((N + 63) >> 6) * S;
      if (s->last_gemm_big_min_tiles > 0 && mid_tiles >= s->last_gemm_big_min_tiles) id |= GK_BODY_128x64;
    }
    *kernel_id = id;
  }
  return TTX_OK;
}

int finish_debug(ttx_session* s, const float* d_slabs, int n_slabs, long long slab_stride, const float* d_bias, const float* d_resid,
                 const float* d_g1, const float* d_b1, const float* d_g2, const float* d_b2, const uint8_t* d_row_valid, float* d_y,
                 const int32_t* d_m, int m_max, int d, float eps, hipStream_t st) {
  if (!s || !d_slabs || !d_bias || !d_resid || !d_g1 || !d_b1 || !d_y) return fail(TTX_ERR_INVALID, "null argument to ttx_debug_finish_ln");
  if ((d_g2 == nullptr) != (d_b2 == nullptr)) return fail(TTX_ERR_INVALID, "ttx_debug_finish_ln: the second norm needs both gamma and beta");
  if (d != 64 && d != 128 && d != 256 && d != 512 && d != 1024) return fail(TTX_ERR_INVALID, "ttx_debug_finish_ln: d must be 64, 128, 256, 512 or 1024");
  if (m_max <= 0 || n_slabs < 1 || !(eps >= 0.f)) return fail(TTX_ERR_INVALID, "ttx_debug_finish_ln: m_max and n_slabs must be positive, eps >= 0");
  if (n_slabs > 1 && (slab_stride < (long long)m_max * d || (slab_stride & 3)))
    return fail(TTX_ERR_INVALID, "ttx_debug_finish_ln: slab_stride must cover one [m_max, d] slab and be a multiple of 4");
  for (const void* p : {(const void*)d_slabs, (const void*)d_bias, (const void*)d_resid, (const void*)d_g1, (const void*)d_b1,
                        (const void*)d_g2, (const void*)d_b2, (const void*)d_y})
    if (!aligned16(p)) return fail(TTX_ERR_INVALID, "ttx_debug_finish_ln: float operands must be 16-byte aligned");
  HIP_TRY(hipSetDevice(s->m->device));
  int M = 0;
  TTX_TRY(debug_live_rows(d_m, m_max, st, &M));
  return launch_finish_d(st, d_slabs, n_slabs, slab_stride, d_bias, d_resid, d_g1, d_b1, d_g2, d_b2, d_row_valid, d_y, d_m, m_max, d, eps);
}

}
```

### translation-transformer_amd/csrc/ttx_internal.h

```cpp
#pragma once
#include "ttx.h"
#include "ttx_common.hip.h"

#include <map>
#include <set>
#include <string>
#include <utility>
#include <vector>

namespace ttx {
struct BeamHost;
struct BeamPoolHost;
}

struct LayerW {
  size_t sa_in_w, sa_in_b, sa_out_w, sa_out_b;
  size_t ca_in_w, ca_in_b, ca_out_w, ca_out_b;
  size_t l1_w, l1_b, l2_w, l2_b;
  size_t n1_w, n1_b, n2_w, n2_b, n3_w, n3_b;
};

struct ttx_model {
  ttx_config cfg;
  int device;
  int activation = TTX_ACT_RELU;
  int n_sessions = 0;

  int n_cu = 256;
  float* blob = nullptr;
  size_t blob_floats = 0;
  std::map<std::string, std::pair<size_t, size_t>> index;
  std::vector<LayerW> enc, dec;
  size_t src_emb, tgt_emb, enc_norm_w, enc_norm_b, dec_norm_w, dec_norm_b, cls_w, cls_b, pe;
  size_t cross_kv_w, cross_kv_b;
  const float* p(size_t off) const { return blob + off; }
};

struct Buf {
  void* p = nullptr;
  size_t cap = 0;
  uint64_t* owner_gen = nullptr;
  template <typename T> T* as() const { return reinterpret_cast<T*>(p); }
};

enum GemmVariant { GV_BIG = 0, GV_SMALL = 1, GV_BIG_FFN2_SLABS = 2, GV_MID = 3 };

enum GemmKernelId { GK_GEMM3 = 1, GK_GEMM_TN = 2, GK_GEMM24_4 = 3, GK_GEMM24_0 = 4, GK_GEMM2_1 = 5, GK_GEMM2_2 = 6, GK_GEMM2_4 = 7,
                    GK_GEMM2_0 = 8, GK_BODY_128x64 = 16 };

enum AttnKernelId { AK_ATTN = 1, AK_ATTN2 = 2, AK_ATTN3 = 3, AK_ATTN3S = 4, AK_ATTN1 = 5 };

enum GraphSite { GS_STEP_SPECULATIVE = 0, GS_STEP_GREEDY = 1, GS_STEP_ROW_RULE = 2, GS_STEP_POOL = 3, GS_BEAM_ITER = 4, GS_BEAM_POOL_ITER = 5,
                 GS_STEP_SAMPLE = 6, GS_STEP_SAMPLE_SPEC = 7, GS_STEP_POOL_SAMPLE = 8,
                 GS_STEP_SAMPLE_PREFIX = 9, GS_STEP_SAMPLE_SPEC_PREFIX = 10, GS_STEP_POOL_SAMPLE_PREFIX = 11,
                 GS_STEP_SAMPLE_SPEC_PROPOSAL = 12, GS_STEP_POOL_SAMPLE_PROPOSAL = 13, GS_SBS_POOL_ITER = 14,
                 GS_LOGIT_BIAS = 256 };
typedef std::vector<int> GraphKey;

struct GraphCache {
  std::map<GraphKey, hipGraphExec_t> map;
  std::set<GraphKey> warmed;
  size_t limit;
  explicit GraphCache(size_t limit_) : limit(limit_) {}
  void clear() {
    for (auto& kv : map) (void)hipGraphExecDestroy(kv.second);
    map.clear(); warmed.clear();
  }
};

#define TTX_SESSION_BUFS(X)                                                                                                      \
                                                                      \
  X(x) X(x1) X(x2) X(xf) X(ao) X(q2) X(hbuf) X(slab) X(qkv) X(logits) X(ckv)                                                      \
                                                                                                                    \
  X(tok_src) X(src_valid) X(memory) X(memkv)                                                                                     \
                                                                                                               \
  X(tok_tgt) X(mem_pad_tmp)                                                                                                      \
   \
  X(ev_logits) X(ev_pred) X(ev_nll)                                                                                              \
   \
                                                                                                      \
  X(sc_src_of) X(am_length)                                                                                                                   \
                                    \
  X(lq_tok)                                                                                                                      \
                                                                                                                       \
  X(drafts) X(gen) X(front) X(act_idx) X(rec) X(pred) X(state) X(kcache) X(vcache) X(src32) X(outbuf) X(haspad) X(traj)           \
  X(fin_step)                                                                                                                    \
                                                                                            \
  X(rstep) X(row_of) X(src_len) X(new_slot) X(pool_io) X(memkv_new) X(valid_new) X(drafts_new)                                    \
       \
            \
  X(qkv_probe) X(pred_probe) X(pred_draft) X(act2) X(pos2) X(state2)                                                             \
         \
  X(draft_mask) X(row_base) X(row_map)                                                                                           \
                           \
  X(accept_blk)                                                                                                                  \
                                        \
  X(snap_logits) X(snap_act) X(snap_front) X(snap_gen) X(snap_state)                                                             \
  X(leaf_score) X(leaf_tok) X(leaf_cnt) X(beam_summary)                                                                          \
                                                                                               \
  X(bs_cand_next) X(bs_len_next) X(bs_fin_next) X(bs_logp_next) X(bs_len) X(bs_fin) X(bs_active) X(bs_logp) X(bs_per_cand)        \
  X(bs_best_n) X(bs_best_slot) X(bs_chosen) X(bs_parent) X(bs_parent_draft) X(bs_mark) X(bs_drafts_src) X(bs_cnt) X(bs_hit)       \
                                                                                 \
  X(t_prev_len) X(t_slot_of) X(t_src_of)                                                                                         \
                                            \
  X(bp_row_of) X(bp_batch) X(bp_cand) X(bp_cand_len) X(bp_tok) X(bp_new_slot) X(bp_io) X(bp_grp) X(bp_src_acc) X(bp_enc_qkv)            \
   \
                     \
  X(smp_key) X(smp_sample) X(smp_done) X(smp_src_of) X(smp_prm) X(smp_drafts)                                                     \
   \
       \
  X(pfx_tok) X(pfx_len_src) X(pfx_len) X(pfx_src) X(pfx_draft0)                                                                  \
   \
                                                              \
  X(lb_val) X(lb_src)                                                                                                            \
    \
  X(sbs_g) X(sbs_g_next)                                                                                                         \
   \
                                                                                          \
  X(sbp_slot) X(sbp_len) X(sbp_io)
#define TTX_DECLARE_BUF(name) Buf name;
#define TTX_REGISTER_BUF(name) all.push_back(&name);

#ifndef TTX_BIG_MIN_TILES
#define TTX_BIG_MIN_TILES 400
#endif
struct ttx_session {
  ttx_model* m;
  std::vector<Buf*> all;
  TTX_SESSION_BUFS(TTX_DECLARE_BUF)
  Buf tk[2], tv[2];
  int snap_B = 0, snap_rps = 0, snap_gen_ld = 0, snap_step = 0;
  ttx::ProbeInfo* probe_info = nullptr;
  long long pool_counters[7] = {};
  long long logit_bias_launches = 0;
  ttx::BeamHost* beam_host = nullptr;
  ttx::BeamPoolHost* bp_host = nullptr;
  ttx::HostInfo* host_info = nullptr;
  hipStream_t own_stream = nullptr;
  uint64_t alloc_generation = 0;
  uint64_t graphs_generation = 0;
  bool dead = false;
  bool use_graphs = true;
  GraphCache step_graphs{512};
  GraphCache iter_graphs{256};
  hipEvent_t ev_done = nullptr;
  void drop_graphs() { step_graphs.clear(); iter_graphs.clear(); }
  void graphs_current() { if (graphs_generation != alloc_generation) { drop_graphs(); graphs_generation = alloc_generation; } }
  ttx::DecState* host_state = nullptr;
  bool attr_attn2[2][8] = {};
  bool attr_select = false, attr_step = false, attr_topk = false, attr_pool_select = false, attr_sbs_step = false;
  bool attr_sbs_step_masked[5] = {};
  bool attr_sbs_step_pool = false, attr_sbs_step_pool_masked[5] = {};
  bool attr_attn_probs[8] = {};
  int qkv_small_rows = 800;
  int small_rows = 2000;
  int ffn2_slab_rows = 5600;
  int big_min_tiles = TTX_BIG_MIN_TILES;
  int last_gemm_kernel = 0, last_gemm_big_min_tiles = 0;
  int attn_split = -1;
  int attn_row = -1;
  bool accept_spread = true;
  bool attn_fallback = false;
  int attn_force = 0;
  int attn_sel_N = 0, attn_sel_D = 0;
  int last_attn_kernel = 0;
  unsigned attn_kernels_seen = 0;
  bool profile = false;
  std::vector<std::pair<hipEvent_t, hipEvent_t>> ev_pool;
  size_t ev_used = 0;
  double prof_ms = 0;
  double prof_empty_pair_ms = -1;
  long long prof_launches = 0;
  bool host_timing = false;
  double host_launch_us = 0;
  long long host_captures = 0;
  double host_capture_us = 0;
  long long host_launches = 0;
  hipEvent_t ev_a = nullptr, ev_b = nullptr, ev_c = nullptr;
  ttx_session() {
    TTX_SESSION_BUFS(TTX_REGISTER_BUF)
    for (Buf* b : {&tk[0], &tk[1], &tv[0], &tv[1]}) all.push_back(b);
    for (Buf* b : all) b->owner_gen = &alloc_generation;
  }
};

namespace ttx {

int fail(int code, const std::string& msg);

#define HIP_TRY(expr)                                                                                  \
  do {                                                                                                 \
    hipError_t _e = (expr);                                                                            \
    if (_e != hipSuccess)                                                                              \
      return ttx::fail(TTX_ERR_HIP, std::string(#expr) + ": " + hipGetErrorString(_e) + " (" __FILE__ ":" + \
                                        std::to_string(__LINE__) + ")");                               \
  } while (0)

#define TTX_TRY(expr)        \
  do {                       \
    int _r = (expr);         \
    if (_r != TTX_OK) return _r; \
  } while (0)

static inline int cdiv(int a, int b) { return (a + b - 1) / b; }

int gemm_slice_k(int K);
int gemm_splits(int N, int K, bool step, int variant);
int launch_gemm(ttx_session* s, hipStream_t st, const float* X, int ldx, const float* W, int ldw, const float* bias,
                float* Y, int ldy, const int* m_ptr, int Mmax, int N, int K, int act, int splits, long long slab_stride,
                int variant);
int launch_finish(ttx_session* s, hipStream_t st, const float* slabs, int n_slabs, long long slab_stride, const float* bias,
                  const float* resid, const float* g1, const float* b1, const float* g2, const float* b2,
                  const uint8_t* row_valid, float* Y, const int* m_ptr, int Mmax);
int launch_finish_d(hipStream_t st, const float* slabs, int n_slabs, long long slab_stride, const float* bias, const float* resid,
                    const float* g1, const float* b1, const float* g2, const float* b2, const uint8_t* row_valid, float* Y,
                    const int* m_ptr, int Mmax, int d, float eps);
int gemm_debug(ttx_session* s, const float* d_x, int ldx, const float* d_w, int ldw, const float* d_bias, float* d_y, int ldy,
               const int32_t* d_m, int m_max, int N, int K, int act, int splits, long long slab_stride, int variant, int tiling,
               int32_t* kernel_id, hipStream_t st);
int finish_debug(ttx_session* s, const float* d_slabs, int n_slabs, long long slab_stride, const float* d_bias, const float* d_resid,
                 const float* d_g1, const float* d_b1, const float* d_g2, const float* d_b2, const uint8_t* d_row_valid, float* d_y,
                 const int32_t* d_m, int m_max, int d, float eps, hipStream_t st);
int gemm_bench(ttx_session* s, int M, int N, int K, int splits, int variant, int reps, double* us_per_launch, double* max_abs_diff);

int launch_attn(int mode, ttx_session* s, hipStream_t st, const AttnArgs& a, int groups, int H, int q_per_group, int max_keys,
                int N = 1, int D1 = 1);
int attn_debug(ttx_session* s, const AttnArgs& in, int H, int head_dim, int mode, int groups, int n_active, int max_keys, int kernel,
               int32_t* kernel_id, hipStream_t st);
int attn_staged_key_limit(int head_dim, int q_per_group);

}
```

### translation-transformer_amd/model.py

```python
from __future__ import annotations

import ctypes as C
import os
import math
from typing import NamedTuple

import numpy as np
import torch

from . import _native as N


def reference_pe_table(emb: int, max_len: int = 5000) -> torch.Tensor:
    pe = torch.zeros(max_len, emb)
    position = torch.arange(0, max_len, dtype=torch.float).unsqueeze(1)
    div_term = torch.exp(torch.arange(0, emb, 2).float() * (-math.log(10000.0) / emb))
    pe[:, 0::2] = torch.sin(position * div_term)
    pe[:, 1::2] = torch.cos(position * div_term)
    return torch.vstack((torch.zeros(1, emb), pe)).contiguous()


def _strip(state: dict) -> dict:
    if any(k.startswith("model.") for k in state):
        return {k[len("model."):]: v for k, v in state.items() if k.startswith("model.")}
# ... 104 lines not shown
            arr[i] = N.Tensor(name, C.cast(v.data_ptr(), C.POINTER(C.c_float)), v.numel())
        N.check(self._lib.ttx_model_create(C.byref(self.cfg), arr, len(host), dev.index or 0, C.byref(self._model)))
        N.check(self._lib.ttx_model_set_activation(self._model, act))
        N.check(self._lib.ttx_session_create(self._model, C.byref(self._session)))

    def blob_tensor(self) -> torch.Tensor:
        ptr, nbytes = C.c_void_p(), C.c_int64()
        N.check(self._lib.ttx_model_blob(self._model, C.byref(ptr), C.byref(nbytes)))
        with torch.cuda.device(self.device):
            t = torch.as_tensor(_DeviceSpan(int(ptr.value), int(nbytes.value)), device=self.device)
        t._ttx_owner = self
        return t

    def _stream(self) -> C.c_void_p:
        return C.c_void_p(torch.cuda.current_stream(self.device).cuda_stream)

    @property
    def session(self) -> C.c_void_p:
        return self._session

    def new_session(self) -> C.c_void_p:
        s = C.c_void_p()
        had = os.environ.get("TTX_PROFILE_GEMM")
        if self._profile_sessions:
            os.environ["TTX_PROFILE_GEMM"] = "1"
        try:
            N.check(self._lib.ttx_session_create(self._model, C.byref(s)))
        finally:
            if self._profile_sessions:
                if had is None:
                    os.environ.pop("TTX_PROFILE_GEMM", None)
                else:
                    os.environ["TTX_PROFILE_GEMM"] = had
        return s

    def session_pool(self, n: int) -> list:
        pool = getattr(self, "_pool", None)
        if pool is None:
            pool = self._pool = [self._session]
        while len(pool) < n:
            pool.append(self.new_session())
        return pool[:n]

    def kernel_profile(self) -> dict:
        ms, n, e = C.c_double(), C.c_int64(), C.c_double()
        tot_ms, tot_n, over, lb = 0.0, 0, [], 0
        for sess in (getattr(self, "_pool", None) or [self._session]):
            lb += int(self._lib.ttx_debug_logit_bias_launches(sess))
            N.check(self._lib.ttx_last_kernel_profile(sess, C.byref(ms), C.byref(n), C.byref(e)))
            tot_ms += ms.value
            tot_n += n.value
            if n.value and e.value > 0:
                over.append(e.value)
        return {"gemm_ms": tot_ms, "launches": tot_n, "pair_overhead_ms": float(np.median(over)) if over else 0.0,
                "logit_bias_launches": lb}

    @staticmethod
    def _ptr(t: torch.Tensor | None):
        return None if t is None else t.data_ptr()

    def debug_gemm(self, x: torch.Tensor, w: torch.Tensor, bias: torch.Tensor | None, y: torch.Tensor, n: int, k: int,
                   m_max: int, m_live: torch.Tensor | None = None, relu: bool = False, splits: int = 0, slab_stride: int = 0,
                   variant: int = 0, tiling: int = 0, activation: int | None = None) -> int:
        kid = C.c_int32(0)
        if activation is not None:
            N.check(self._lib.ttx_debug_gemm_act(self._session, x.data_ptr(), x.stride(0), w.data_ptr(), w.stride(0), self._ptr(bias),
                                                 y.data_ptr(), y.stride(0), self._ptr(m_live), int(m_max), int(n), int(k),
                                                 int(activation), int(splits), int(slab_stride), int(variant), int(tiling),
                                                 C.byref(kid), self._stream()))
            return int(kid.value)
        N.check(self._lib.ttx_debug_gemm(self._session, x.data_ptr(), x.stride(0), w.data_ptr(), w.stride(0), self._ptr(bias),
                                         y.data_ptr(), y.stride(0), self._ptr(m_live), int(m_max), int(n), int(k), int(relu),
                                         int(splits), int(slab_stride), int(variant), int(tiling), C.byref(kid), self._stream()))
        return int(kid.value)

    def debug_finish_ln(self, slabs: torch.Tensor, n_slabs: int, slab_stride: int, bias: torch.Tensor, resid: torch.Tensor,
                        g1: torch.Tensor, b1: torch.Tensor, g2: torch.Tensor | None, b2: torch.Tensor | None,
                        row_valid: torch.Tensor | None, y: torch.Tensor, m_max: int, d: int, eps: float = 1e-5,
                        m_live: torch.Tensor | None = None) -> None:
        N.check(self._lib.ttx_debug_finish_ln(self._session, slabs.data_ptr(), int(n_slabs), int(slab_stride), bias.data_ptr(),
                                              resid.data_ptr(), g1.data_ptr(), b1.data_ptr(), self._ptr(g2), self._ptr(b2),
                                              self._ptr(row_valid), y.data_ptr(), self._ptr(m_live), int(m_max), int(d),
                                              float(eps), self._stream()))

    def debug_attn(self, mode: int, q: torch.Tensor, k: torch.Tensor, v: torch.Tensor, out: torch.Tensor, heads: int, scale: float,
                   groups: int, max_keys: int, L: int = 0, Lk: int = 0, tok: torch.Tensor | None = None, pad: int = 0,
                   key_pad: torch.Tensor | None = None, mem_row: torch.Tensor | None = None, act_idx: torch.Tensor | None = None,
                   front: torch.Tensor | None = None, src_of: torch.Tensor | None = None, src_len: torch.Tensor | None = None,
                   kcache: torch.Tensor | None = None, vcache: torch.Tensor | None = None, cache_seq_stride: int = 0,
                   cache_slot: torch.Tensor | None = None, gen_ld: int = 0, n: int = 1, d: int = 0, n_active: int = 0,
                   kernel: int = 0, head_dim: int = 32, choose_as: tuple | None = None) -> int:
        kid = C.c_int32(0)
        assert k.stride(0) == v.stride(0)
        if choose_as is not None:
            N.check(self._lib.ttx_debug_attn_as(self._session, q.data_ptr(), q.stride(0), k.data_ptr(), v.data_ptr(), k.stride(0),
                                                out.data_ptr(), int(heads), int(head_dim), float(scale), int(L), int(Lk), self._ptr(tok),
                                                int(pad), self._ptr(key_pad), self._ptr(mem_row), self._ptr(act_idx), self._ptr(front),
                                                self._ptr(src_of), self._ptr(src_len), self._ptr(kcache), self._ptr(vcache),
                                                int(cache_seq_stride), self._ptr(cache_slot), int(gen_ld), int(n), int(d), int(mode),
                                                int(groups), int(n_active), int(max_keys), int(kernel), C.byref(kid),
                                                int(choose_as[0]), int(choose_as[1]), self._stream()))
            return int(kid.value)
        N.check(self._lib.ttx_debug_attn_hd(self._session, q.data_ptr(), q.stride(0), k.data_ptr(), v.data_ptr(), k.stride(0),
                                            out.data_ptr(), int(heads), int(head_dim), float(scale), int(L), int(Lk), self._ptr(tok),
                                            int(pad), self._ptr(key_pad), self._ptr(mem_row), self._ptr(act_idx), self._ptr(front),
                                            self._ptr(src_of), self._ptr(src_len), self._ptr(kcache), self._ptr(vcache),
                                            int(cache_seq_stride), self._ptr(cache_slot), int(gen_ld), int(n), int(d), int(mode),
                                            int(groups), int(n_active), int(max_keys), int(kernel), C.byref(kid), self._stream()))
        return int(kid.value)

    def debug_attn_probs(self, q: torch.Tensor, k: torch.Tensor, key_pad: torch.Tensor, length: torch.Tensor, heads: int,
                         head_dim: int, T: int, Ls: int, scale: float, mem_row: torch.Tensor | None = None,
                         out_heads: torch.Tensor | None = None, out_mean: torch.Tensor | None = None,
                         out_align: torch.Tensor | None = None) -> None:
        R, Rm = int(length.numel()), int(key_pad.numel()) // int(Ls)
        N.check(self._lib.ttx_debug_attn_probs(self._session, q.data_ptr(), q.stride(0), k.data_ptr(), k.stride(0), key_pad.data_ptr(),
                                               self._ptr(mem_row), length.data_ptr(), R, Rm, int(heads), int(head_dim), int(T), int(Ls),
                                               float(scale), self._ptr(out_heads), self._ptr(out_mean), self._ptr(out_align),
                                               self._stream()))

    @staticmethod
    def attn_probs_key_limit(head_dim: int) -> int:
        return int(N.lib().ttx_attn_probs_key_limit(int(head_dim)))

    def debug_argmax(self, logits: torch.Tensor, pred: torch.Tensor, m_max: int, m_live: torch.Tensor | None = None) -> None:
        N.check(self._lib.ttx_debug_argmax(self._session, logits.data_ptr(), int(logits.shape[1]), pred.data_ptr(),
                                           self._ptr(m_live), int(m_max), self._stream()))

    def debug_logit_bias(self, logits: torch.Tensor, bias: torch.Tensor, src: torch.Tensor | None = None, m_live: torch.Tensor | None = None,
                         rows_per_src: int = 1, act_idx: torch.Tensor | None = None, row_map: torch.Tensor | None = None, n: int = 1,
                         d: int = 0) -> None:
        M, V = logits.shape
        assert logits.stride(1) == 1 and logits.stride(0) == V and bias.stride(1) == 1
        N.check(self._lib.ttx_debug_logit_bias(self.session, logits.data_ptr(), V, M, self._ptr(m_live), bias.data_ptr(),
                                               int(bias.stride(0)), self._ptr(src), rows_per_src, self._ptr(act_idx), self._ptr(row_map),
                                               n, d, self._stream()))

    def debug_sample(self, logits: torch.Tensor, key: torch.Tensor, sample: torch.Tensor, done: torch.Tensor, front: torch.Tensor,
                     pred: torch.Tensor, m_max: int, m_live: torch.Tensor | None = None, *, temperature: float = 1.0, top_k: int = 0,
                     top_p: float = 1.0, pad: int = 0, eos: int = 2, seed: int = 0) -> None:
        p = N.SampleParams(1, 1, float(temperature), int(top_k), float(top_p), int(pad), 0, int(eos), int(seed) & 0xFFFFFFFFFFFFFFFF)
        N.check(self._lib.ttx_debug_sample(self._session, logits.data_ptr(), int(logits.shape[1]), key.data_ptr(), sample.data_ptr(),
                                           done.data_ptr(), front.data_ptr(), pred.data_ptr(), self._ptr(m_live), int(m_max),
                                           C.byref(p), self._stream()))

    def debug_sample_step(self, logits: torch.Tensor, key: torch.Tensor, sample: torch.Tensor, act_idx: torch.Tensor,
                          front: torch.Tensor, pred: torch.Tensor, *, B: int, n: int, d: int, n_active: int,
                          m_live: torch.Tensor | None = None, temperature: float = 1.0, top_k: int = 0, top_p: float = 1.0,
                          pad: int = 0, eos: int = 2, seed: int = 0) -> None:
        p = N.SampleParams(1, 1, float(temperature), int(top_k), float(top_p), int(pad), 0, int(eos), int(seed) & 0xFFFFFFFFFFFFFFFF)
        N.check(self._lib.ttx_debug_sample_step(self._session, logits.data_ptr(), int(logits.shape[1]), key.data_ptr(),
                                                sample.data_ptr(), act_idx.data_ptr(), front.data_ptr(), int(B), int(n), int(d),
                                                int(n_active), pred.data_ptr(), self._ptr(m_live), C.byref(p), self._stream()))

    def debug_embed(self, table: torch.Tensor, pe: torch.Tensor, x: torch.Tensor, tok: torch.Tensor | None = None, rows: int = 0,
                    L: int = 0, act_idx: torch.Tensor | None = None, front: torch.Tensor | None = None,
                    gen: torch.Tensor | None = None, drafts: torch.Tensor | None = None, B: int = 0, n: int = 1, d: int = 0,
                    n_active: int = 0, step: bool = False) -> None:
        N.check(self._lib.ttx_debug_embed(self._session, table.data_ptr(), int(table.shape[0]), pe.data_ptr(), int(pe.shape[0]),
                                          int(table.shape[1]), x.data_ptr(), self._ptr(tok), int(rows), int(L), self._ptr(act_idx),
                                          self._ptr(front), self._ptr(gen), 0 if gen is None else int(gen.stride(0)),
                                          self._ptr(drafts), int(B), int(n), int(d), int(n_active), int(bool(step)), self._stream()))

    def debug_accept(self, state, *, B: int, n: int, d: int, Ls: int, max_len: int, pad: int, bos: int, eos: int, gen_ld: int,
                     greedy: bool = False, threads: int = 0, row_rule: bool = False, pool: bool = False, traj_ld: int = 0,
                     pool_rows: int = 0, _entry: str = "ttx_debug_accept", **arrays) -> list:
# ... 761 lines not shown
```

Baseline: 23930.

## Fuse split-K LayerNorm finish into the prologue of the next decoder GEMM

Adds a k_gemm3_ln path in which the next small GEMM (cross-attn query, FFN1, next layer QKV, classifier) reduces the previous GEMM's split-K slabs, applies bias, residual and LayerNorm, writes the normalized rows, and then multiplies. The decoder stack defers each finish launch instead of issuing it separately. This is enabled by default for d=256 step decoding (ln_prologue=-1 with rows threshold 0 means always on) and aims to cut kernel launches and an extra round trip through memory per LN. In exchange, several GEMM blocks may redundantly recompute LN for the same rows, and the kernel becomes more complex.

```diff
diff --git a/include/ttx.h b/include/ttx.h
--- a/include/ttx.h
+++ b/include/ttx.h
@@ -350,6 +350,17 @@
                         const float* d_resid, const float* d_g1, const float* d_b1, const float* d_g2, const float* d_b2,
                         const uint8_t* d_row_valid, float* d_y, const int32_t* d_m, int m_max, int d, float eps, void* stream);
 
+int ttx_debug_gemm_ln(ttx_session* s, const float* d_slabs, int n_slabs, int64_t slab_stride, const float* d_fbias,
+                      const float* d_resid, const float* d_g1, const float* d_b1, const float* d_g2, const float* d_b2,
+                      const uint8_t* d_row_valid, float* d_y_ln, int d, float eps, const float* d_w, int ldw, const float* d_bias,
+                      float* d_y, int ldy, const int32_t* d_m, int m_max, int N, int K, int activation, int32_t* kernel_id,
+                      void* stream);
+
+int ttx_debug_gemm_ln_bench(ttx_session* s, int M, int N, int n_slabs, int variant, int reps, double* us_fused, double* us_pair,
+                            double* max_abs_diff);
+
+int ttx_debug_ln_fused_launches(ttx_session* s);
+
 int ttx_debug_attn(ttx_session* s, const float* d_q, int ldq, const float* d_k, const float* d_v, int ldkv, float* d_out, int H,
                    float scale, int L, int Lk, const int32_t* d_tok, int pad, const uint8_t* d_key_pad, const int32_t* d_mem_row,
                    const int32_t* d_act_idx, const int32_t* d_front, const int32_t* d_src_of, const int32_t* d_src_len,
diff --git a/translation-transformer_amd/_native.py b/translation-transformer_amd/_native.py
--- a/translation-transformer_amd/_native.py
+++ b/translation-transformer_amd/_native.py
@@ -327,6 +327,10 @@
     "ttx_debug_gemm_act": (C.c_int, [_VP, _VP, _I, _VP, _I, _VP, _VP, _I, _VP, _I, _I, _I, _I, _I, C.c_int64, _I, _I,
                                      C.POINTER(C.c_int32), _VP]),
     "ttx_debug_finish_ln": (C.c_int, [_VP, _VP, _I, C.c_int64, _VP, _VP, _VP, _VP, _VP, _VP, _VP, _VP, _VP, _I, _I, C.c_float, _VP]),
+    "ttx_debug_gemm_ln": (C.c_int, [_VP, _VP, _I, C.c_int64, _VP, _VP, _VP, _VP, _VP, _VP, _VP, _VP, _I, C.c_float, _VP, _I, _VP, _VP, _I,
+                                    _VP, _I, _I, _I, _I, C.POINTER(C.c_int32), _VP]),
+    "ttx_debug_gemm_ln_bench": (C.c_int, [_VP, _I, _I, _I, _I, _I, C.POINTER(C.c_double), C.POINTER(C.c_double), C.POINTER(C.c_double)]),
+    "ttx_debug_ln_fused_launches": (C.c_int, [_VP]),
     "ttx_debug_attn": (C.c_int, [_VP, _VP, _I, _VP, _VP, _I, _VP, _I, C.c_float, _I, _I, _VP, _I, _VP, _VP, _VP, _VP, _VP, _VP, _VP, _VP,
                                  C.c_int64, _VP, _I, _I, _I, _I, _I, _I, _I, _I, C.POINTER(C.c_int32), _VP]),
     "ttx_debug_attn_hd": (C.c_int, [_VP, _VP, _I, _VP, _VP, _I, _VP, _I, _I, C.c_float, _I, _I, _VP, _I, _VP, _VP, _VP, _VP, _VP, _VP, _VP,
diff --git a/translation-transformer_amd/csrc/ttx_api.hip b/translation-transformer_amd/csrc/ttx_api.hip
--- a/translation-transformer_amd/csrc/ttx_api.hip
+++ b/translation-transformer_amd/csrc/ttx_api.hip
@@ -314,6 +314,10 @@
   if (const char* e = getenv("TTX_SMALL_ROWS")) s->small_rows = std::max(0, atoi(e));
   if (const char* e = getenv("TTX_FFN2_SLAB_ROWS")) s->ffn2_slab_rows = std::max(0, atoi(e));
   if (const char* e = getenv("TTX_QKV_SMALL_ROWS")) s->qkv_small_rows = std::max(0, atoi(e));
+  if (const char* e = getenv("TTX_LN_PROLOGUE")) s->ln_prologue = atoi(e) != 0 ? 1 : 0;
+  if (const char* e = getenv("TTX_LN_PROLOGUE_ROWS")) s->ln_prologue_rows = std::max(0, atoi(e));
+  if (const char* e = getenv("TTX_LN_FFN1_ROWS")) s->ln_ffn1_rows = std::max(0, atoi(e));
+  if (m->cfg.embedding_dim != 256) s->ln_prologue = 0;
   if (const char* e = getenv("TTX_ATTN_FALLBACK")) s->attn_fallback = atoi(e) != 0;
   if (const char* e = getenv("TTX_ACCEPT_SPREAD")) s->accept_spread = atoi(e) != 0;
   if (const char* e = getenv("TTX_ATTN_ROW")) s->attn_row = atoi(e) != 0 ? 1 : 0;
@@ -356,33 +360,40 @@
 
 static int variant_for_rows(const ttx_session* s, long long rows, bool step) {
   if (!step) return GV_BIG;
-  if (rows < s->qkv_small_rows) return GV_SMALL;
-  if (rows < s->small_rows) return GV_MID;
-  return rows < s->ffn2_slab_rows ? GV_BIG_FFN2_SLABS : GV_BIG;
-}
-static int variant_qkv(int v) { return v == GV_SMALL ? GV_SMALL : GV_BIG; }
-static int variant_dd(int v) { return (v == GV_SMALL || v == GV_MID) ? GV_SMALL : GV_BIG; }
-static int variant_ffn1(int v) { return v == GV_SMALL ? GV_SMALL : GV_BIG; }
-static int variant_ffn2(int v) { return v == GV_BIG ? GV_BIG : GV_SMALL; }
+  const int gv = rows < s->qkv_small_rows ? GV_SMALL : rows < s->small_rows ? GV_MID : rows < s->ffn2_slab_rows ? GV_BIG_FFN2_SLABS : GV_BIG;
+  if (s->ln_prologue == 0 || (s->ln_prologue < 0 && rows >= s->ln_prologue_rows)) return gv;
+  return gv | GVF_LN_PROLOGUE | ((gv == GV_SMALL && rows < s->ln_ffn1_rows) ? GVF_LN_FFN1 : 0);
+}
+static int variant_qkv(int v) { return (v & GV_MASK) == GV_SMALL ? GV_SMALL : GV_BIG; }
+static int variant_dd(int v) { v &= GV_MASK; return (v == GV_SMALL || v == GV_MID) ? GV_SMALL : GV_BIG; }
+static int variant_ffn1(int v) { return (v & GV_MASK) == GV_SMALL ? GV_SMALL : GV_BIG; }
+static int variant_ffn2(int v) { return (v & GV_MASK) == GV_BIG ? GV_BIG : GV_SMALL; }
 
 static int gemm_ln(ttx_session* s, hipStream_t st, const float* X, int ldx, int K, const float* W, const float* bias,
                    const float* resid, const float* g1, const float* b1, const float* g2, const float* b2,
-                   const uint8_t* row_valid, float* Y, const int* m_ptr, int Mmax, int variant) {
+                   const uint8_t* row_valid, float* Y, const int* m_ptr, int Mmax, int variant, FinishArgs* defer = nullptr) {
   const int d = s->m->cfg.embedding_dim;
   const int S = gemm_splits(d, K, m_ptr != nullptr, variant);
   const long long stride = (long long)Mmax * d;
   TTX_TRY(ensure(s->slab, sizeof(float) * (size_t)S * stride, st));
   TTX_TRY(launch_gemm(s, st, X, ldx, W, K, nullptr, s->slab.as<float>(), d, m_ptr, Mmax, d, K, false, S, stride, variant));
+  if (defer) {
+    FinishArgs& f = *defer;
+    f.slabs = s->slab.as<float>(); f.n_slabs = S; f.slab_stride = stride; f.bias = bias; f.resid = resid; f.g1 = g1; f.b1 = b1;
+    f.g2 = g2; f.b2 = b2; f.row_valid = row_valid; f.Y = Y; f.m_ptr = m_ptr; f.M = Mmax; f.d = d; f.eps = s->m->cfg.layer_norm_eps;
+    return TTX_OK;
+  }
   return launch_finish(s, st, s->slab.as<float>(), S, stride, bias, resid, g1, b1, g2, b2, row_valid, Y, m_ptr, Mmax);
 }
 
 static int ffn_half(ttx_session* s, hipStream_t st, const LayerW& w, const float* x, size_t n_w, size_t n_b, const float* g2,
-                    const float* b2, const uint8_t* row_valid, float* Y, const int* m_ptr, int Mmax, int v_ffn1, int v_ffn2) {
+                    const float* b2, const uint8_t* row_valid, float* Y, const int* m_ptr, int Mmax, int v_ffn1, int v_ffn2,
+                    const FinishArgs* pend_x = nullptr, FinishArgs* defer = nullptr) {
   const ttx_model* m = s->m;
   const int d = m->cfg.embedding_dim, F = m->cfg.feedforward_dim;
   float* hb = s->hbuf.as<float>();
-  TTX_TRY(launch_gemm(s, st, x, d, m->p(w.l1_w), d, m->p(w.l1_b), hb, F, m_ptr, Mmax, F, d, m->activation, 0, 0, v_ffn1));
-  return gemm_ln(s, st, hb, F, F, m->p(w.l2_w), m->p(w.l2_b), x, m->p(n_w), m->p(n_b), g2, b2, row_valid, Y, m_ptr, Mmax, v_ffn2);
+  TTX_TRY(launch_gemm(s, st, x, d, m->p(w.l1_w), d, m->p(w.l1_b), hb, F, m_ptr, Mmax, F, d, m->activation, 0, 0, v_ffn1, pend_x));
+  return gemm_ln(s, st, hb, F, F, m->p(w.l2_w), m->p(w.l2_b), x, m->p(n_w), m->p(n_b), g2, b2, row_valid, Y, m_ptr, Mmax, v_ffn2, defer);
 }
 
 static int ensure_acts(ttx_session* s, hipStream_t st, size_t M, int qkv_layers) {
@@ -483,6 +494,7 @@
   const int* m_ptr;
   int Mmax;
   int v_qkv, v_dd, v_ffn1, v_ffn2;
+  bool defer_ln = false;
   float* qkv;
   long long qkv_layer;
 };
@@ -499,23 +511,28 @@
   float* xf = s->xf.as<float>();
   float* ao = s->ao.as<float>();
   float* q2 = s->q2.as<float>();
+  const bool defer = r.defer_ln && r.m_ptr != nullptr && d == 256 && stop_layer < 0;
+  FinishArgs pend;
+  FinishArgs* to_pend = defer ? &pend : nullptr;
+  const FinishArgs* from_x = nullptr;
   for (int l = 0; l < Ld; ++l) {
     const LayerW& w = m->dec[l];
     const bool last = (l == Ld - 1);
     float* qkv = r.qkv + (size_t)l * r.qkv_layer;
-    TTX_TRY(launch_gemm(s, st, x, d, m->p(w.sa_in_w), d, m->p(w.sa_in_b), qkv, 3 * d, r.m_ptr, r.Mmax, 3 * d, d, false, 0, 0, r.v_qkv));
+    TTX_TRY(launch_gemm(s, st, x, d, m->p(w.sa_in_w), d, m->p(w.sa_in_b), qkv, 3 * d, r.m_ptr, r.Mmax, 3 * d, d, false, 0, 0, r.v_qkv, from_x));
     TTX_TRY(self_attn(l, qkv));
     TTX_TRY(gemm_ln(s, st, ao, d, d, m->p(w.sa_out_w), m->p(w.sa_out_b), x, m->p(w.n1_w), m->p(w.n1_b), nullptr, nullptr,
-                    nullptr, x1, r.m_ptr, r.Mmax, r.v_dd));
-    TTX_TRY(launch_gemm(s, st, x1, d, m->p(w.ca_in_w), d, m->p(w.ca_in_b), q2, d, r.m_ptr, r.Mmax, d, d, false, 0, 0, r.v_dd));
+                    nullptr, x1, r.m_ptr, r.Mmax, r.v_dd, to_pend));
+    TTX_TRY(launch_gemm(s, st, x1, d, m->p(w.ca_in_w), d, m->p(w.ca_in_b), q2, d, r.m_ptr, r.Mmax, d, d, false, 0, 0, r.v_dd, to_pend));
     TTX_TRY(cross_attn(l));
     if (l == stop_layer) return TTX_OK;
     TTX_TRY(gemm_ln(s, st, ao, d, d, m->p(w.ca_out_w), m->p(w.ca_out_b), x1, m->p(w.n2_w), m->p(w.n2_b), nullptr, nullptr,
-                    nullptr, x2, r.m_ptr, r.Mmax, r.v_dd));
+                    nullptr, x2, r.m_ptr, r.Mmax, r.v_dd, to_pend));
     TTX_TRY(ffn_half(s, st, w, x2, w.n3_w, w.n3_b, last ? m->p(m->dec_norm_w) : nullptr, last ? m->p(m->dec_norm_b) : nullptr,
-                     nullptr, last ? xf : x, r.m_ptr, r.Mmax, r.v_ffn1, r.v_ffn2));
-  }
-  return launch_gemm(s, st, xf, d, m->p(m->cls_w), d, m->p(m->cls_b), logits, V, r.m_ptr, r.Mmax, V, d, false, 0, 0, r.v_dd);
+                     nullptr, last ? xf : x, r.m_ptr, r.Mmax, r.v_ffn1, r.v_ffn2, to_pend, to_pend));
+    from_x = to_pend;
+  }
+  return launch_gemm(s, st, xf, d, m->p(m->cls_w), d, m->p(m->cls_b), logits, V, r.m_ptr, r.Mmax, V, d, false, 0, 0, r.v_dd, from_x);
 }
 
 struct AttnTap {
@@ -545,7 +562,7 @@
   e.table = m->p(m->tgt_emb); e.pe = m->p(m->pe); e.X = s->x.as<float>(); e.d = d; e.V = c.vocab_size; e.tok = tok; e.rows = M; e.L = Lt;
   hipLaunchKernelGGL((k_embed<false>), dim3(cdiv(M, 4)), dim3(256), 0, st, e);
   HIP_TRY(hipGetLastError());
-  const StackRows rows{nullptr, M, gv, gv, gv, gv, s->qkv.as<float>(), 0};
+  const StackRows rows{nullptr, M, gv, gv, gv, gv, false, s->qkv.as<float>(), 0};
   return run_decoder_stack(s, st, rows,
       [&](int, float* qkv) -> int {
         AttnArgs a{};
@@ -1082,8 +1099,9 @@
   hipLaunchKernelGGL((k_embed<true>), dim3(cdiv(Mmax, 4)), dim3(256), 0, st, e);
   HIP_TRY(hipGetLastError());
 
-  const StackRows rows{m_ptr, Mmax, variant_qkv(k.variant), variant_dd(k.variant), variant_ffn1(k.variant), variant_ffn2(k.variant),
-                       k.qkv_ov ? k.qkv_ov : s->qkv.as<float>(), (long long)Mmax * 3 * d};
+  const StackRows rows{m_ptr, Mmax, variant_qkv(k.variant), variant_dd(k.variant),
+                       variant_ffn1(k.variant) | ((k.variant & GVF_LN_FFN1) ? GVF_GEMM3_WIDE : 0), variant_ffn2(k.variant),
+                       (k.variant & GVF_LN_PROLOGUE) != 0, k.qkv_ov ? k.qkv_ov : s->qkv.as<float>(), (long long)Mmax * 3 * d};
   TTX_TRY(run_decoder_stack(s, st, rows,
       [&](int l, float* qkv) -> int {
         AttnArgs a{};
@@ -3827,6 +3845,24 @@
                             slab_stride, variant, tiling, kernel_id, stream);
 }
 
+extern "C" int ttx_debug_gemm_ln(ttx_session* s, const float* d_slabs, int n_slabs, int64_t slab_stride, const float* d_fbias,
+                                 const float* d_resid, const float* d_g1, const float* d_b1, const float* d_g2, const float* d_b2,
+                                 const uint8_t* d_row_valid, float* d_y_ln, int d, float eps, const float* d_w, int ldw,
+                                 const float* d_bias, float* d_y, int ldy, const int32_t* d_m, int m_max, int N, int K, int activation,
+                                 int32_t* kernel_id, void* stream) {
+  return gemm_ln_debug(s, d_slabs, n_slabs, (long long)slab_stride, d_fbias, d_resid, d_g1, d_b1, d_g2, d_b2, d_row_valid, d_y_ln, d, eps,
+                       d_w, ldw, d_bias, d_y, ldy, d_m, m_max, N, K, activation, kernel_id, reinterpret_cast<hipStream_t>(stream));
+}
+
+extern "C" int ttx_debug_gemm_ln_bench(ttx_session* s, int M, int N, int n_slabs, int variant, int reps, double* us_fused,
+                                       double* us_pair, double* max_abs_diff) {
+  return gemm_ln_bench(s, M, N, n_slabs, variant, reps, us_fused, us_pair, max_abs_diff);
+}
+
+extern "C" int ttx_debug_ln_fused_launches(ttx_session* s) {
+  return s ? (int)std::min<long long>(s->ln_fused_launches, 0x7fffffff) : 0;
+}
+
 extern "C" int ttx_debug_finish_ln(ttx_session* s, const float* d_slabs, int n_slabs, int64_t slab_stride, const float* d_bias,
                                    const float* d_resid, const float* d_g1, const float* d_b1, const float* d_g2, const float* d_b2,
                                    const uint8_t* d_row_valid, float* d_y, const int32_t* d_m, int m_max, int d, float eps,
diff --git a/translation-transformer_amd/csrc/ttx_gemm.hip b/translation-transformer_amd/csrc/ttx_gemm.hip
--- a/translation-transformer_amd/csrc/ttx_gemm.hip
+++ b/translation-transformer_amd/csrc/ttx_gemm.hip
@@ -513,32 +513,17 @@
   }
 }
 
-template <bool GELU = false>
-__global__ __launch_bounds__(256) __attribute__((amdgpu_waves_per_eu(1, 4))) void k_gemm3(GemmArgs a) {
-  constexpr int KW = 64;
-  __shared__ __attribute__((aligned(16))) float part[4][32 * 33];
-  const int M = a.m_ptr ? *a.m_ptr : a.M;
-  const int m0 = blockIdx.y * 32, n0 = blockIdx.x * 32;
-  if (m0 >= M) return;
-  const int t = threadIdx.x, wave = t >> 6, lane = t & 63;
-  const int r = lane & 31, h = lane >> 5;
-  const int kbeg = blockIdx.z * a.k_per_split + wave * KW;
-  const float* xp = a.X + (size_t)min(m0 + r, M - 1) * a.ldx + kbeg + 4 * h;
-  const float* wp = a.W + (size_t)min(n0 + r, a.N - 1) * a.ldw + kbeg + 4 * h;
+typedef float f32x4 __attribute__((ext_vector_type(4)));
+constexpr int G3_KW = 64;
+
+template <bool GELU>
+__device__ __forceinline__ void gemm3_tile(const GemmArgs& a, int M, int m0, int n0, int t, int wave, int r, int h,
+                                           const f32x4 (&av)[G3_KW / 8], const f32x4 (&bv)[G3_KW / 8], float (*part)[32 * 33]) {
   f32x16 acc;
 #pragma unroll
   for (int i = 0; i < 16; ++i) acc[i] = 0.f;
-  typedef float f32x4 __attribute__((ext_vector_type(4)));
-  f32x4 av[KW / 8], bv[KW / 8];
-#pragma unroll
-  for (int g = 0; g < KW / 8; ++g) {
-    av[g] = *reinterpret_cast<const f32x4*>(xp + 8 * g);
-    bv[g] = *reinterpret_cast<const f32x4*>(wp + 8 * g);
-  }
-  asm volatile("" : "+v"(av[0]), "+v"(av[1]), "+v"(av[2]), "+v"(av[3]), "+v"(av[4]), "+v"(av[5]), "+v"(av[6]), "+v"(av[7]),
-                    "+v"(bv[0]), "+v"(bv[1]), "+v"(bv[2]), "+v"(bv[3]), "+v"(bv[4]), "+v"(bv[5]), "+v"(bv[6]), "+v"(bv[7]));
-#pragma unroll
-  for (int g = 0; g < KW / 8; ++g) {
+#pragma unroll
+  for (int g = 0; g < G3_KW / 8; ++g) {
     acc = __builtin_amdgcn_mfma_f32_32x32x2f32(av[g].x, bv[g].x, acc, 0, 0, 0);
     acc = __builtin_amdgcn_mfma_f32_32x32x2f32(av[g].y, bv[g].y, acc, 0, 0, 0);
     acc = __builtin_amdgcn_mfma_f32_32x32x2f32(av[g].z, bv[g].z, acc, 0, 0, 0);
@@ -573,6 +558,29 @@
   }
 }
 
+template <bool GELU = false>
+__global__ __launch_bounds__(256) __attribute__((amdgpu_waves_per_eu(1, 4))) void k_gemm3(GemmArgs a) {
+  constexpr int KW = G3_KW;
+  __shared__ __attribute__((aligned(16))) float part[4][32 * 33];
+  const int M = a.m_ptr ? *a.m_ptr : a.M;
+  const int m0 = blockIdx.y * 32, n0 = blockIdx.x * 32;
+  if (m0 >= M) return;
+  const int t = threadIdx.x, wave = t >> 6, lane = t & 63;
+  const int r = lane & 31, h = lane >> 5;
+  const int kbeg = blockIdx.z * a.k_per_split + wave * KW;
+  const float* xp = a.X + (size_t)min(m0 + r, M - 1) * a.ldx + kbeg + 4 * h;
+  const float* wp = a.W + (size_t)min(n0 + r, a.N - 1) * a.ldw + kbeg + 4 * h;
+  f32x4 av[KW / 8], bv[KW / 8];
+#pragma unroll
+  for (int g = 0; g < KW / 8; ++g) {
+    av[g] = *reinterpret_cast<const f32x4*>(xp + 8 * g);
+    bv[g] = *reinterpret_cast<const f32x4*>(wp + 8 * g);
+  }
+  asm volatile("" : "+v"(av[0]), "+v"(av[1]), "+v"(av[2]), "+v"(av[3]), "+v"(av[4]), "+v"(av[5]), "+v"(av[6]), "+v"(av[7]),
+                    "+v"(bv[0]), "+v"(bv[1]), "+v"(bv[2]), "+v"(bv[3]), "+v"(bv[4]), "+v"(bv[5]), "+v"(bv[6]), "+v"(bv[7]));
+  gemm3_tile<GELU>(a, M, m0, n0, t, wave, r, h, av, bv, part);
+}
+
 template <int VPL>
 __device__ __forceinline__ void ln_inplace(float (&x)[VPL], const float* g, const float* b, int c0, int d, float eps) {
   float s = 0.f;
@@ -586,6 +594,113 @@
   const float rstd = 1.0f / sqrtf(var + eps);
 #pragma unroll
   for (int i = 0; i < VPL; ++i) x[i] = (x[i] - mean) * rstd * g[c0 + i] + b[c0 + i];
+}
+
+struct Finish4Par { float4 b4, g1, e1, g2, e2; };
+template <int NS> struct Finish4In { float4 r4, t0, p[NS > 1 ? NS - 1 : 1]; uint8_t valid; };
+
+__device__ __forceinline__ Finish4Par finish4_par(const FinishArgs& a, int c0) {
+  Finish4Par q;
+  q.b4 = *reinterpret_cast<const float4*>(a.bias + c0);
+  q.g1 = *reinterpret_cast<const float4*>(a.g1 + c0);
+  q.e1 = *reinterpret_cast<const float4*>(a.b1 + c0);
+  const float* g2p = a.g2 ? a.g2 : a.g1;
+  const float* e2p = a.g2 ? a.b2 : a.b1;
+  q.g2 = *reinterpret_cast<const float4*>(g2p + c0);
+  q.e2 = *reinterpret_cast<const float4*>(e2p + c0);
+  return q;
+}
+
+template <int NS>
+__device__ __forceinline__ void finish4_load(const FinishArgs& a, int row, int c0, Finish4In<NS>& in) {
+  const size_t off = (size_t)row * a.d + c0;
+  in.r4 = *reinterpret_cast<const float4*>(a.resid + off);
+  in.t0 = *reinterpret_cast<const float4*>(a.slabs + off);
+#pragma unroll
+  for (int s = 0; s < NS - 1; ++s) in.p[s] = *reinterpret_cast<const float4*>(a.slabs + (size_t)(s + 1) * a.slab_stride + off);
+  in.valid = a.row_valid ? a.row_valid[row] : (uint8_t)1;
+}
+
+template <int NS>
+__device__ __forceinline__ void finish4_row(const FinishArgs& a, const Finish4Par& q, const Finish4In<NS>& in, float (&x)[4]) {
+  float4 tsum = in.t0;
+#pragma unroll
+  for (int s = 0; s < NS - 1; ++s) { tsum.x += in.p[s].x; tsum.y += in.p[s].y; tsum.z += in.p[s].z; tsum.w += in.p[s].w; }
+  x[0] = (in.r4.x + q.b4.x) + tsum.x; x[1] = (in.r4.y + q.b4.y) + tsum.y; x[2] = (in.r4.z + q.b4.z) + tsum.z; x[3] = (in.r4.w + q.b4.w) + tsum.w;
+  const float ga[4] = {q.g1.x, q.g1.y, q.g1.z, q.g1.w}, ea[4] = {q.e1.x, q.e1.y, q.e1.z, q.e1.w};
+  ln_inplace<4>(x, ga, ea, 0, a.d, a.eps);
+  if (a.g2) {
+    const float gb[4] = {q.g2.x, q.g2.y, q.g2.z, q.g2.w}, eb[4] = {q.e2.x, q.e2.y, q.e2.z, q.e2.w};
+    ln_inplace<4>(x, gb, eb, 0, a.d, a.eps);
+  }
+  if (in.valid == 0) { x[0] = 0.f; x[1] = 0.f; x[2] = 0.f; x[3] = 0.f; }
+}
+
+template <int R>
+__device__ __forceinline__ void pin_rows(float (&v)[R]) {
+  static_assert(R == 4 || R == 8, "batches of 4 or 8 rows");
+  if constexpr (R == 8) asm volatile("" : "+v"(v[0]), "+v"(v[1]), "+v"(v[2]), "+v"(v[3]), "+v"(v[4]), "+v"(v[5]), "+v"(v[6]), "+v"(v[7]));
+  else asm volatile("" : "+v"(v[0]), "+v"(v[1]), "+v"(v[2]), "+v"(v[3]));
+}
+
+template <int R>
+__device__ __forceinline__ void wave_sum_rows(float (&v)[R]) {
+  pin_rows<R>(v);
+#pragma unroll
+  for (int o = 32; o > 0; o >>= 1) {
+    float t[R];
+#pragma unroll
+    for (int i = 0; i < R; ++i) t[i] = __shfl_xor(v[i], o, 64);
+    pin_rows<R>(t);
+#pragma unroll
+    for (int i = 0; i < R; ++i) v[i] += t[i];
+    pin_rows<R>(v);
+  }
+}
+
+template <int R>
+__device__ __forceinline__ void ln4_rows(float (&x)[R][4], const float4& g4, const float4& e4, int d, float eps) {
+  const float g[4] = {g4.x, g4.y, g4.z, g4.w}, b[4] = {e4.x, e4.y, e4.z, e4.w};
+  float s[R], q[R];
+#pragma unroll
+  for (int i = 0; i < R; ++i) {
+    s[i] = 0.f;
+#pragma unroll
+    for (int k = 0; k < 4; ++k) s[i] += x[i][k];
+  }
+  wave_sum_rows<R>(s);
+#pragma unroll
+  for (int i = 0; i < R; ++i) {
+    s[i] = s[i] / (float)d;
+    q[i] = 0.f;
+#pragma unroll
+    for (int k = 0; k < 4; ++k) { const float t = x[i][k] - s[i]; q[i] += t * t; }
+  }
+  wave_sum_rows<R>(q);
+#pragma unroll
+  for (int i = 0; i < R; ++i) {
+    const float var = q[i] / (float)d;
+    const float rstd = 1.0f / sqrtf(var + eps);
+#pragma unroll
+    for (int k = 0; k < 4; ++k) x[i][k] = (x[i][k] - s[i]) * rstd * g[k] + b[k];
+  }
+}
+
+template <int NS, int R>
+__device__ __forceinline__ void finish4_rows(const FinishArgs& a, const Finish4Par& q, const Finish4In<NS> (&in)[R], float (&x)[R][4]) {
+#pragma unroll
+  for (int i = 0; i < R; ++i) {
+    float4 tsum = in[i].t0;
+#pragma unroll
+    for (int s = 0; s < NS - 1; ++s) { tsum.x += in[i].p[s].x; tsum.y += in[i].p[s].y; tsum.z += in[i].p[s].z; tsum.w += in[i].p[s].w; }
+    x[i][0] = (in[i].r4.x + q.b4.x) + tsum.x; x[i][1] = (in[i].r4.y + q.b4.y) + tsum.y;
+    x[i][2] = (in[i].r4.z + q.b4.z) + tsum.z; x[i][3] = (in[i].r4.w + q.b4.w) + tsum.w;
+  }
+  ln4_rows<R>(x, q.g1, q.e1, a.d, a.eps);
+  if (a.g2) ln4_rows<R>(x, q.g2, q.e2, a.d, a.eps);
+#pragma unroll
+  for (int i = 0; i < R; ++i)
+    if (in[i].valid == 0) { x[i][0] = 0.f; x[i][1] = 0.f; x[i][2] = 0.f; x[i][3] = 0.f; }
 }
 
 template <int VPL>
@@ -645,6 +760,64 @@
   for (int i = 0; i < VPL; ++i) a.Y[off + i] = keep ? x[i] : 0.f;
 }
 
+constexpr int G3_PANEL_LD = 256 + 4;
+template <bool GELU, int NS>
+__global__ __launch_bounds__(256) void k_gemm3_ln(GemmArgs a, FinishArgs f) {
+  constexpr int KW = G3_KW;
+  __shared__ __attribute__((aligned(16))) float part[4][32 * 33];
+  __shared__ __attribute__((aligned(16))) float panel[32 * G3_PANEL_LD];
+  const int M = a.m_ptr ? *a.m_ptr : a.M;
+  const int m0 = blockIdx.y * 32, n0 = blockIdx.x * 32;
+  if (m0 >= M) return;
+  const int t = threadIdx.x, wave = t >> 6, lane = t & 63;
+  const int r = lane & 31, h = lane >> 5;
+  const float* wp = a.W + (size_t)min(n0 + r, a.N - 1) * a.ldw + wave * KW + 4 * h;
+  f32x4 av[KW / 8], bv[KW / 8];
+#pragma unroll
+  for (int g = 0; g < KW / 8; ++g) bv[g] = *reinterpret_cast<const f32x4*>(wp + 8 * g);
+  const int c0 = lane * 4;
+  const bool store_ln = blockIdx.x == 0;
+  auto put = [&](int j, const float (&x)[4]) {
+    const float4 v = make_float4(x[0], x[1], x[2], x[3]);
+    *reinterpret_cast<float4*>(&panel[j * G3_PANEL_LD + c0]) = v;
+    if (store_ln && m0 + j < M) *reinterpret_cast<float4*>(f.Y + (size_t)(m0 + j) * 256 + c0) = v;
+  };
+  if constexpr (NS > 0) {
+    constexpr int RB = NS == 1 ? 8 : 4;
+    const Finish4Par q = finish4_par(f, c0);
+#pragma unroll
+    for (int b = 0; b < 8; b += RB) {
+      Finish4In<NS> in[RB];
+#pragma unroll
+      for (int i = 0; i < RB; ++i) finish4_load<NS>(f, min(m0 + wave + 4 * (b + i), M - 1), c0, in[i]);
+      float x[RB][4];
+      finish4_rows<NS, RB>(f, q, in, x);
+#pragma unroll
+      for (int i = 0; i < RB; ++i) put(wave + 4 * (b + i), x[i]);
+    }
+  } else {
+    const Finish4Par q = finish4_par(f, c0);
+    for (int i = 0; i < 8; ++i) {
+      const int row = min(m0 + wave + 4 * i, M - 1);
+      Finish4In<1> in;
+      finish4_load<1>(f, row, c0, in);
+      for (int s = 1; s < f.n_slabs; ++s) {
+        const float4 p = *reinterpret_cast<const float4*>(f.slabs + (size_t)s * f.slab_stride + (size_t)row * 256 + c0);
+        in.t0.x += p.x; in.t0.y += p.y; in.t0.z += p.z; in.t0.w += p.w;
+      }
+      float x[4];
+      finish4_row<1>(f, q, in, x);
+      put(wave + 4 * i, x);
+    }
+  }
+  __syncthreads();
+#pragma unroll
+  for (int g = 0; g < KW / 8; ++g) av[g] = *reinterpret_cast<const f32x4*>(&panel[r * G3_PANEL_LD + wave * KW + 8 * g + 4 * h]);
+  asm volatile("" : "+v"(av[0]), "+v"(av[1]), "+v"(av[2]), "+v"(av[3]), "+v"(av[4]), "+v"(av[5]), "+v"(av[6]), "+v"(av[7]),
+                    "+v"(bv[0]), "+v"(bv[1]), "+v"(bv[2]), "+v"(bv[3]), "+v"(bv[4]), "+v"(bv[5]), "+v"(bv[6]), "+v"(bv[7]));
+  gemm3_tile<GELU>(a, M, m0, n0, t, wave, r, h, av, bv, part);
+}
+
 
 int gemm_slice_k(int K) {
   if (K == 64 || K == 128) return 64;
@@ -652,19 +825,24 @@
   return K >= 2048 ? 256 : 64;
 }
 
-static bool use_gemm3(bool step, int variant, int N, int K) {
-  return step && variant == GV_SMALL && K == 256 && N <= 768;
-}
+static bool use_gemm3(bool step, int variant, int N, int K, bool wide = false) {
+  return step && variant == GV_SMALL && K == 256 && (N <= 768 || (wide && N <= G3_WIDE_MAX_N));
+}
+
+static bool ranges_overlap(const float* p, size_t n, const float* q, size_t m) { return p < q + m && q < p + n; }
 
 int gemm_splits(int N, int K, bool step, int variant) {
   (void)N;
+  variant &= GV_MASK;
   if (step && variant == GV_SMALL && gemm_slice_k(K) == 256 && K / 256 <= 16) return K / 256;
   return 1;
 }
 
 int launch_gemm(ttx_session* s, hipStream_t st, const float* X, int ldx, const float* W, int ldw, const float* bias,
                 float* Y, int ldy, const int* m_ptr, int Mmax, int N, int K, int act, int splits, long long slab_stride,
-                int variant) {
+                int variant, const FinishArgs* pend) {
+  const bool wide = (variant & GVF_GEMM3_WIDE) != 0;
+  variant &= GV_MASK;
   if (act != TTX_ACT_NONE && act != TTX_ACT_RELU && act != TTX_ACT_GELU) return fail(TTX_ERR_INVALID, "GEMM activation must be a ttx_activation");
   if (Mmax <= 0) return TTX_OK;
   if (K % 32) return fail(TTX_ERR_INVALID, "GEMM K must be a multiple of 32");
@@ -683,6 +861,22 @@
     return fail(TTX_ERR_INVALID, "split-K slabs must be 64, 128 or a multiple of 256 deep");
   if (!a.slice_k && a.k_per_split % 32) return fail(TTX_ERR_INVALID, "split-K slabs must be a multiple of 32 deep");
   a.big_min_tiles = 0;
+  const bool step = (m_ptr != nullptr);
+  bool fused = false;
+  if (pend) {
+    if (pend->Y != X || ldx != pend->d || pend->m_ptr != m_ptr || pend->M != Mmax)
+      return fail(TTX_ERR_INVALID, "a pending finisher must produce the GEMM's X rows");
+    fused = use_gemm3(step, variant, N, K, wide) && S == 1 && pend->d == 256;
+    if (fused) {
+      const size_t rows = (size_t)Mmax * 256;
+      if (ranges_overlap(pend->Y, rows, pend->resid, rows) ||
+          ranges_overlap(pend->Y, rows, pend->slabs, (size_t)(pend->n_slabs - 1) * pend->slab_stride + rows))
+        return fail(TTX_ERR_INVALID, "k_gemm3_ln: the finished rows must not alias the residual or the slabs");
+    } else {
+      TTX_TRY(launch_finish_d(st, pend->slabs, pend->n_slabs, pend->slab_stride, pend->bias, pend->resid, pend->g1, pend->b1, pend->g2,
+                              pend->b2, pend->row_valid, pend->Y, m_ptr, Mmax, pend->d, pend->eps));
+    }
+  }
   hipEvent_t e1 = nullptr;
   if (s->profile) {
     if (s->ev_used == s->ev_pool.size()) {
@@ -695,10 +889,24 @@
     e1 = s->ev_pool[s->ev_used].second;
     s->ev_used++;
   }
-  const bool step = (m_ptr != nullptr);
   const bool gelu = act == TTX_ACT_GELU;
   s->last_gemm_big_min_tiles = 0;
-  if (use_gemm3(step, variant, N, K) && S == 1) {
+  if (fused) {
+    s->last_gemm_kernel = GK_GEMM3_LN;
+    s->ln_fused_launches += 1;
+    const dim3 grid(cdiv(N, 32), cdiv(Mmax, 32), 1);
+    const int ns = (pend->n_slabs == 1 || pend->n_slabs == 8) ? pend->n_slabs : 0;
+    if (gelu) switch (ns) {
+      case 1: hipLaunchKernelGGL((k_gemm3_ln<true, 1>), grid, dim3(256), 0, st, a, *pend); break;
+      case 8: hipLaunchKernelGGL((k_gemm3_ln<true, 8>), grid, dim3(256), 0, st, a, *pend); break;
+      default: hipLaunchKernelGGL((k_gemm3_ln<true, 0>), grid, dim3(256), 0, st, a, *pend); break;
+    }
+    else switch (ns) {
+      case 1: hipLaunchKernelGGL((k_gemm3_ln<false, 1>), grid, dim3(256), 0, st, a, *pend); break;
+      case 8: hipLaunchKernelGGL((k_gemm3_ln<false, 8>), grid, dim3(256), 0, st, a, *pend); break;
+      default: hipLaunchKernelGGL((k_gemm3_ln<false, 0>), grid, dim3(256), 0, st, a, *pend); break;
+    }
+  } else if (use_gemm3(step, variant, N, K, wide) && S == 1) {
     s->last_gemm_kernel = GK_GEMM3;
     if (gelu) hipLaunchKernelGGL((k_gemm3<true>), dim3(cdiv(N, 32), cdiv(Mmax, 32), 1), dim3(256), 0, st, a);
     else hipLaunchKernelGGL((k_gemm3<false>), dim3(cdiv(N, 32), cdiv(Mmax, 32), 1), dim3(256), 0, st, a);
@@ -916,4 +1124,130 @@
   return launch_finish_d(st, d_slabs, n_slabs, slab_stride, d_bias, d_resid, d_g1, d_b1, d_g2, d_b2, d_row_valid, d_y, d_m, m_max, d, eps);
 }
 
-}
+int gemm_ln_debug(ttx_session* s, const float* d_slabs, int n_slabs, long long slab_stride, const float* d_fbias, const float* d_resid,
+                  const float* d_g1, const float* d_b1, const float* d_g2, const float* d_b2, const uint8_t* d_row_valid, float* d_y_ln,
+                  int d, float eps, const float* d_w, int ldw, const float* d_bias, float* d_y, int ldy, const int32_t* d_m, int m_max,
+                  int N, int K, int act, int32_t* kernel_id, hipStream_t st) {
+  if (!s || !d_slabs || !d_fbias || !d_resid || !d_g1 || !d_b1 || !d_y_ln || !d_w || !d_y || !d_m)
+    return fail(TTX_ERR_INVALID, "null argument to ttx_debug_gemm_ln");
+  if ((d_g2 == nullptr) != (d_b2 == nullptr)) return fail(TTX_ERR_INVALID, "ttx_debug_gemm_ln: the second norm needs both gamma and beta");
+  if (act != TTX_ACT_NONE && act != TTX_ACT_RELU && act != TTX_ACT_GELU) return fail(TTX_ERR_INVALID, "ttx_debug_gemm_ln: activation is 0 (none), 1 (ReLU) or 2 (GELU)");
+  if (K != 256 || d != 256) return fail(TTX_ERR_INVALID, "ttx_debug_gemm_ln: k_gemm3_ln serves K = d = 256");
+  if (N <= 0 || N % 32 || N > G3_WIDE_MAX_N) return fail(TTX_ERR_INVALID, "ttx_debug_gemm_ln: N must be a multiple of 32, at most 2048");
+  if (m_max <= 0 || n_slabs < 1 || n_slabs > 16 || !(eps >= 0.f)) return fail(TTX_ERR_INVALID, "ttx_debug_gemm_ln: m_max positive, 1..16 slabs, eps >= 0");
+  if (ldw < K || (ldw & 3) || ldy < N) return fail(TTX_ERR_INVALID, "ttx_debug_gemm_ln: ldw must cover K and be a multiple of 4, ldy must cover N");
+  const size_t rows = (size_t)m_max * 256;
+  if (n_slabs > 1 && (slab_stride < (long long)rows || (slab_stride & 3)))
+    return fail(TTX_ERR_INVALID, "ttx_debug_gemm_ln: slab_stride must cover one [m_max, d] slab and be a multiple of 4");
+  for (const void* p : {(const void*)d_slabs, (const void*)d_fbias, (const void*)d_resid, (const void*)d_g1, (const void*)d_b1,
+                        (const void*)d_g2, (const void*)d_b2, (const void*)d_y_ln, (const void*)d_w, (const void*)d_bias})
+    if (!aligned16(p)) return fail(TTX_ERR_INVALID, "ttx_debug_gemm_ln: float operands must be 16-byte aligned");
+  if ((ldy & 3) == 0 && !aligned16(d_y)) return fail(TTX_ERR_INVALID, "ttx_debug_gemm_ln: Y must be 16-byte aligned when ldy is a multiple of 4");
+  const size_t slab_span = (size_t)(n_slabs - 1) * (size_t)slab_stride + rows;
+  if (ranges_overlap(d_y_ln, rows, d_resid, rows) || ranges_overlap(d_y_ln, rows, d_slabs, slab_span) ||
+      ranges_overlap(d_y_ln, rows, d_y, (size_t)(m_max - 1) * ldy + N))
+    return fail(TTX_ERR_INVALID, "ttx_debug_gemm_ln: d_y_ln must not alias the residual, the slabs or Y");
+  HIP_TRY(hipSetDevice(s->m->device));
+  int M = 0;
+  TTX_TRY(debug_live_rows(d_m, m_max, st, &M));
+  FinishArgs f;
+  f.slabs = d_slabs; f.n_slabs = n_slabs; f.slab_stride = slab_stride; f.bias = d_fbias; f.resid = d_resid; f.g1 = d_g1; f.b1 = d_b1;
+  f.g2 = d_g2; f.b2 = d_b2; f.row_valid = d_row_valid; f.Y = d_y_ln; f.m_ptr = d_m; f.M = m_max; f.d = d; f.eps = eps;
+  const bool was_profile = s->profile;
+  const long long keep_count = s->ln_fused_launches;
+  s->profile = false;
+  const int rc = launch_gemm(s, st, d_y_ln, 256, d_w, ldw, d_bias, d_y, ldy, d_m, m_max, N, K, act, 0, 0, GV_SMALL | GVF_GEMM3_WIDE, &f);
+  s->profile = was_profile;
+  s->ln_fused_launches = keep_count;
+  if (rc != TTX_OK) return rc;
+  if (s->last_gemm_kernel != GK_GEMM3_LN) return fail(TTX_ERR_INVALID, "ttx_debug_gemm_ln: the launch did not reach k_gemm3_ln");
+  if (kernel_id) *kernel_id = s->last_gemm_kernel;
+  return TTX_OK;
+}
+
+int gemm_ln_bench(ttx_session* s, int M, int N, int n_slabs, int variant, int reps, double* us_fused, double* us_pair, double* max_abs_diff) {
+  if (!s || M <= 0 || N <= 0 || N % 32 || N > G3_WIDE_MAX_N || n_slabs < 1 || n_slabs > 16 || reps <= 0 || variant < GV_BIG || variant > GV_MID)
+    return fail(TTX_ERR_INVALID, "bad argument to ttx_debug_gemm_ln_bench");
+  HIP_TRY(hipSetDevice(s->m->device));
+  const int d = 256;
+  const size_t rows = (size_t)M * d;
+  std::vector<float> hs((size_t)n_slabs * rows), hr(rows), hw((size_t)N * d), hb(N), hp(5 * d);
+  uint64_t z = 0x9E3779B97F4A7C15ull;
+  auto rnd = [&]() { z ^= z << 13; z ^= z >> 7; z ^= z << 17; return (float)((z >> 40) & 0xffff) / 65536.f - 0.5f; };
+  for (auto& v : hs) v = rnd();
+  for (auto& v : hr) v = rnd();
+  for (auto& v : hw) v = rnd() * 0.125f;
+  for (auto& v : hb) v = rnd();
+  for (auto& v : hp) v = rnd() + 1.f;
+  float *ds = nullptr, *dr = nullptr, *dw = nullptr, *db = nullptr, *dp = nullptr, *dy[2] = {nullptr, nullptr}, *dl[2] = {nullptr, nullptr};
+  int* dm = nullptr;
+  HIP_TRY(hipMalloc(&ds, hs.size() * 4));
+  HIP_TRY(hipMalloc(&dr, hr.size() * 4));
+  HIP_TRY(hipMalloc(&dw, hw.size() * 4));
+  HIP_TRY(hipMalloc(&db, hb.size() * 4));
+  HIP_TRY(hipMalloc(&dp, hp.size() * 4));
+  for (int i = 0; i < 2; ++i) {
+    HIP_TRY(hipMalloc(&dy[i], (size_t)M * N * 4));
+    HIP_TRY(hipMalloc(&dl[i], rows * 4));
+  }
+  HIP_TRY(hipMalloc(&dm, 4));
+  HIP_TRY(hipMemcpy(ds, hs.data(), hs.size() * 4, hipMemcpyHostToDevice));
+  HIP_TRY(hipMemcpy(dr, hr.data(), hr.size() * 4, hipMemcpyHostToDevice));
+  HIP_TRY(hipMemcpy(dw, hw.data(), hw.size() * 4, hipMemcpyHostToDevice));
+  HIP_TRY(hipMemcpy(db, hb.data(), hb.size() * 4, hipMemcpyHostToDevice));
+  HIP_TRY(hipMemcpy(dp, hp.data(), hp.size() * 4, hipMemcpyHostToDevice));
+  HIP_TRY(hipMemcpy(dm, &M, 4, hipMemcpyHostToDevice));
+  hipStream_t st = nullptr;
+  HIP_TRY(hipStreamCreateWithFlags(&st, hipStreamNonBlocking));
+  const bool was_profile = s->profile;
+  const long long keep_count = s->ln_fused_launches;
+  s->profile = false;
+  auto launch = [&](int form) -> int {
+    FinishArgs f;
+    f.slabs = ds; f.n_slabs = n_slabs; f.slab_stride = (long long)rows; f.bias = dp; f.resid = dr; f.g1 = dp + d; f.b1 = dp + 2 * d;
+    f.g2 = nullptr; f.b2 = nullptr; f.row_valid = nullptr; f.Y = dl[form]; f.m_ptr = dm; f.M = M; f.d = d; f.eps = 1e-5f;
+    if (form) return launch_gemm(s, st, dl[form], d, dw, d, db, dy[form], N, dm, M, N, d, TTX_ACT_NONE, 0, 0, GV_SMALL | GVF_GEMM3_WIDE, &f);
+    TTX_TRY(launch_finish_d(st, f.slabs, f.n_slabs, f.slab_stride, f.bias, f.resid, f.g1, f.b1, f.g2, f.b2, f.row_valid, f.Y, dm, M, d, f.eps));
+    return launch_gemm(s, st, dl[form], d, dw, d, db, dy[form], N, dm, M, N, d, TTX_ACT_NONE, 0, 0, variant);
+  };
+  int rc = TTX_OK;
+  hipEvent_t e0 = nullptr, e1 = nullptr;
+  HIP_TRY(hipEventCreate(&e0));
+  HIP_TRY(hipEventCreate(&e1));
+  double us[2] = {0, 0};
+  for (int form = 0; form < 2 && rc == TTX_OK; ++form) {
+    for (int i = 0; i < 3 && rc == TTX_OK; ++i) rc = launch(form);
+    if (rc == TTX_OK && form == 1 && s->last_gemm_kernel != GK_GEMM3_LN) rc = fail(TTX_ERR_INVALID, "the fused form did not reach k_gemm3_ln");
+    if (rc == TTX_OK && form == 0 && s->last_gemm_kernel == GK_GEMM3_LN) rc = fail(TTX_ERR_INVALID, "the two-launch form reached k_gemm3_ln");
+    if (rc != TTX_OK) break;
+    HIP_TRY(hipEventRecord(e0, st));
+    for (int i = 0; i < reps && rc == TTX_OK; ++i) rc = launch(form);
+    HIP_TRY(hipEventRecord(e1, st));
+    HIP_TRY(hipStreamSynchronize(st));
+    float ms = 0.f;
+    HIP_TRY(hipEventElapsedTime(&ms, e0, e1));
+    us[form] = 1e3 * ms / reps;
+  }
+  if (us_pair) *us_pair = us[0];
+  if (us_fused) *us_fused = us[1];
+  if (rc == TTX_OK && max_abs_diff) {
+    double worst = 0;
+    std::vector<float> u, v;
+    for (int which = 0; which < 2; ++which) {
+      const size_t n = which ? rows : (size_t)M * N;
+      u.resize(n); v.resize(n);
+      HIP_TRY(hipMemcpy(u.data(), which ? dl[0] : dy[0], n * 4, hipMemcpyDeviceToHost));
+      HIP_TRY(hipMemcpy(v.data(), which ? dl[1] : dy[1], n * 4, hipMemcpyDeviceToHost));
+      for (size_t i = 0; i < n; ++i) worst = std::max(worst, (double)std::fabs(u[i] - v[i]));
+    }
+    *max_abs_diff = worst;
+  }
+  s->profile = was_profile; s->ln_fused_launches = keep_count;
+  (void)hipEventDestroy(e0); (void)hipEventDestroy(e1);
+  (void)hipStreamDestroy(st);
+  (void)hipFree(ds); (void)hipFree(dr); (void)hipFree(dw); (void)hipFree(db); (void)hipFree(dp); (void)hipFree(dm);
+  for (int i = 0; i < 2; ++i) { (void)hipFree(dy[i]); (void)hipFree(dl[i]); }
+  return rc;
+}
+
+}
diff --git a/translation-transformer_amd/csrc/ttx_internal.h b/translation-transformer_amd/csrc/ttx_internal.h
--- a/translation-transformer_amd/csrc/ttx_internal.h
+++ b/translation-transformer_amd/csrc/ttx_internal.h
@@ -44,9 +44,11 @@
 };
 
 enum GemmVariant { GV_BIG = 0, GV_SMALL = 1, GV_BIG_FFN2_SLABS = 2, GV_MID = 3 };
+enum GemmVariantFlag { GV_MASK = 7, GVF_LN_PROLOGUE = 8, GVF_LN_FFN1 = 16, GVF_GEMM3_WIDE = GVF_LN_FFN1 };
+constexpr int G3_WIDE_MAX_N = 2048;
 
 enum GemmKernelId { GK_GEMM3 = 1, GK_GEMM_TN = 2, GK_GEMM24_4 = 3, GK_GEMM24_0 = 4, GK_GEMM2_1 = 5, GK_GEMM2_2 = 6, GK_GEMM2_4 = 7,
-                    GK_GEMM2_0 = 8, GK_BODY_128x64 = 16 };
+                    GK_GEMM2_0 = 8, GK_GEMM3_LN = 9, GK_BODY_128x64 = 16 };
 
 enum AttnKernelId { AK_ATTN = 1, AK_ATTN2 = 2, AK_ATTN3 = 3, AK_ATTN3S = 4, AK_ATTN1 = 5 };
 
@@ -154,6 +156,10 @@
   bool attr_attn_probs[8] = {};
   int qkv_small_rows = 800;
   int small_rows = 2000;
+  int ln_prologue = -1;
+  int ln_prologue_rows = 0;
+  int ln_ffn1_rows = 0;
+  long long ln_fused_launches = 0;
   int ffn2_slab_rows = 5600;
   int big_min_tiles = TTX_BIG_MIN_TILES;
   int last_gemm_kernel = 0, last_gemm_big_min_tiles = 0;
@@ -208,7 +214,7 @@
 int gemm_splits(int N, int K, bool step, int variant);
 int launch_gemm(ttx_session* s, hipStream_t st, const float* X, int ldx, const float* W, int ldw, const float* bias,
                 float* Y, int ldy, const int* m_ptr, int Mmax, int N, int K, int act, int splits, long long slab_stride,
-                int variant);
+                int variant, const FinishArgs* pend = nullptr);
 int launch_finish(ttx_session* s, hipStream_t st, const float* slabs, int n_slabs, long long slab_stride, const float* bias,
                   const float* resid, const float* g1, const float* b1, const float* g2, const float* b2,
                   const uint8_t* row_valid, float* Y, const int* m_ptr, int Mmax);
@@ -221,6 +227,11 @@
 int finish_debug(ttx_session* s, const float* d_slabs, int n_slabs, long long slab_stride, const float* d_bias, const float* d_resid,
                  const float* d_g1, const float* d_b1, const float* d_g2, const float* d_b2, const uint8_t* d_row_valid, float* d_y,
                  const int32_t* d_m, int m_max, int d, float eps, hipStream_t st);
+int gemm_ln_debug(ttx_session* s, const float* d_slabs, int n_slabs, long long slab_stride, const float* d_fbias, const float* d_resid,
+                  const float* d_g1, const float* d_b1, const float* d_g2, const float* d_b2, const uint8_t* d_row_valid, float* d_y_ln,
+                  int d, float eps, const float* d_w, int ldw, const float* d_bias, float* d_y, int ldy, const int32_t* d_m, int m_max,
+                  int N, int K, int act, int32_t* kernel_id, hipStream_t st);
+int gemm_ln_bench(ttx_session* s, int M, int N, int n_slabs, int variant, int reps, double* us_fused, double* us_pair, double* max_abs_diff);
 int gemm_bench(ttx_session* s, int M, int N, int K, int splits, int variant, int reps, double* us_per_launch, double* max_abs_diff);
 
 int launch_attn(int mode, ttx_session* s, hipStream_t st, const AttnArgs& a, int groups, int H, int q_per_group, int max_keys,
diff --git a/translation-transformer_amd/model.py b/translation-transformer_amd/model.py
--- a/translation-transformer_amd/model.py
+++ b/translation-transformer_amd/model.py
@@ -210,6 +210,22 @@
                                               resid.data_ptr(), g1.data_ptr(), b1.data_ptr(), self._ptr(g2), self._ptr(b2),
                                               self._ptr(row_valid), y.data_ptr(), self._ptr(m_live), int(m_max), int(d),
                                               float(eps), self._stream()))
+
+    def debug_gemm_ln(self, slabs: torch.Tensor, n_slabs: int, slab_stride: int, fbias: torch.Tensor, resid: torch.Tensor,
+                      g1: torch.Tensor, b1: torch.Tensor, g2: torch.Tensor | None, b2: torch.Tensor | None,
+                      row_valid: torch.Tensor | None, y_ln: torch.Tensor, w: torch.Tensor, bias: torch.Tensor | None, y: torch.Tensor,
+                      n: int, m_max: int, m_live: torch.Tensor | None, activation: int = 0, k: int = 256, d: int = 256,
+                      eps: float = 1e-5) -> int:
+        kid = C.c_int32(0)
+        N.check(self._lib.ttx_debug_gemm_ln(self._session, self._ptr(slabs), int(n_slabs), int(slab_stride), self._ptr(fbias),
+                                            self._ptr(resid), self._ptr(g1), self._ptr(b1), self._ptr(g2), self._ptr(b2),
+                                            self._ptr(row_valid), self._ptr(y_ln), int(d), float(eps), self._ptr(w), w.stride(0),
+                                            self._ptr(bias), self._ptr(y), y.stride(0), self._ptr(m_live), int(m_max), int(n), int(k),
+                                            int(activation), C.byref(kid), self._stream()))
+        return int(kid.value)
+
+    def ln_fused_launches(self, session=None) -> int:
+        return int(self._lib.ttx_debug_ln_fused_launches(self._session if session is None else session))
 
     def debug_attn(self, mode: int, q: torch.Tensor, k: torch.Tensor, v: torch.Tensor, out: torch.Tensor, heads: int, scale: float,
                    groups: int, max_keys: int, L: int = 0, Lk: int = 0, tok: torch.Tensor | None = None, pad: int = 0,
```

Measured after the change: 23880. No clear change (-0.2%).
